# cmbant/getdist

Hardware: AMD Instinct MI355X
Metric: 2D KDE densities/sec (triangle, 50 params, 1e+07 samples) (higher is better)
Workload: dtype f64

## Files before the change

### getdist_amd/_lib.py

```python

import ctypes as C
import os
import subprocess

import numpy as np

_HERE = os.path.dirname(os.path.abspath(__file__))
LIB_PATH = os.path.join(_HERE, "csrc", "libgdhip.so")

GD_OK, GD_ERR_BADARG, GD_ERR_NOMEM, GD_ERR_HIP, GD_ERR_EMPTY, GD_ERR_SOLVER, GD_ERR_FFT, GD_ERR_NODEVICE, GD_ERR_TIMEOUT = \
    0, -1, -2, -3, -4, -5, -6, -7, -8


class GdhipError(RuntimeError):
    def __init__(self, code, msg):
        super().__init__("libgdhip error %d: %s" % (code, msg))
        self.code = code


class GdhipTimeout(GdhipError):
    """GD_ERR_TIMEOUT: a collective or the communicator set-up gave up waiting for a peer; the library has aborted and dropped
    the communicator, so the ranks renegotiate over the host application's own channel (parallel.init_library_comm)."""


def build_native(force=False):
    script = os.path.join(_HERE, "csrc", "build.sh")
    if force:
        for f in os.listdir(os.path.join(_HERE, "csrc")):
            if f.endswith(".o") or f.endswith(".so"):
                os.remove(os.path.join(_HERE, "csrc", f))
    subprocess.run(["bash", script], check=True)
    return LIB_PATH


_p = C.c_void_p
_i32, _i64, _f64 = C.c_int32, C.c_int64, C.c_double
_pd = C.POINTER(C.c_double)
_pi32 = C.POINTER(C.c_int32)
_pi64 = C.POINTER(C.c_int64)

SIGNATURES = {
    "gd_device_count": (C.c_int, []),
    "gd_create": (C.c_int, [C.c_int, C.POINTER(_p)]),
    "gd_destroy": (None, [_p]),
    "gd_last_error": (C.c_char_p, [_p]),
    "gd_version": (C.c_char_p, []),
    "gd_device_info": (C.c_int, [_p, _pi64]),
    "gd_sync": (C.c_int, [_p]),
    "gd_dev_alloc": (C.c_int, [_p, _i64, C.POINTER(_p)]),
    "gd_dev_free": (C.c_int, [_p, _p]),
    "gd_memcpy_h2d": (C.c_int, [_p, _p, _p, _i64]),
    "gd_memcpy_d2h": (C.c_int, [_p, _p, _p, _i64]),
    "gd_memcpy_d2h_async": (C.c_int, [_p, _p, _p, _i64]),
    "gd_copy_sync": (C.c_int, [_p]),
    "gd_memcpy_d2d": (C.c_int, [_p, _p, _p, _i64]),
    "gd_memset": (C.c_int, [_p, _p, C.c_int, _i64]),
    "gd_gather_items": (C.c_int, [_p, _p, _p, _pi32, _i32, _i64]),
    "gd_host_alloc": (C.c_int, [_p, _i64, C.POINTER(_p)]),
    "gd_host_free": (C.c_int, [_p, _p]),
    "gd_kde_lag_sums_2d": (C.c_int, [_p, _i32, _i32, _pd, _pi64, _i32, _pd]),
    "gd_autocov_lags_batch": (C.c_int, [_p, _pi32, _i32, _pd, _i64, _i32, _pd]),
    "gd_kde_lag_sums_batch": (C.c_int, [_p, _pi32, _i32, _pd, _pi64, _i32, _pd]),
    "gd_autocov_lags_range_batch": (C.c_int, [_p, _pi32, _i32, _pd, _i64, _i64, _i64, _i32, _pd]),
    "gd_timer_start": (C.c_int, [_p]),
    "gd_timer_stop_ms": (C.c_int, [_p, _pd]),
    "gd_upload": (C.c_int, [_p, _p, _i64, _i64, _i64, _i64, _p]),
    "gd_num_rows": (C.c_int, [_p, _pi64, _pi64]),
    "gd_column_ptr": (C.c_int, [_p, _i64, C.POINTER(_p)]),
    "gd_weight_stats": (C.c_int, [_p, _i64, _i64, _f64, _pd]),
    "gd_col_stats": (C.c_int, [_p, _i64, _i64, _pd]),
    "gd_cov": (C.c_int, [_p, _pi32, _i32, _i64, _i64, _pd, _pd, _pd, _pd]),
    "gd_quantiles": (C.c_int, [_p, _pi32, _i32, _i64, _i64, _pd, _i32, _pd]),
    "gd_quantiles_mm_probe": (C.c_int, [_p, _pi32, _i32, _i64, _i64, _pd, _i32, _pd, _pd, _pd, _pd, C.POINTER(C.c_int32)]),
    "gd_quantiles_mm": (C.c_int, [_p, _pi32, _i32, _i64, _i64, _pd, _i32, _pd, _pd]),
    "gd_autocov_lags": (C.c_int, [_p, _i32, _f64, _i64, _i32, _pd]),
    "gd_kde_lag_sums": (C.c_int, [_p, _i32, _f64, _pi64, _i32, _pd]),
    "gd_hist1d": (C.c_int, [_p, _pi32, _i32, _pd, _pd, _i32, _pd]),
    "gd_hist1d_dev": (C.c_int, [_p, _pi32, _i32, _pd, _pd, _i32, _p]),
    "gd_bin_indices": (C.c_int, [_p, _i32, _f64, _f64, _i32, _i32, _pi32, _pi64]),
    "gd_prebin": (C.c_int, [_p, _i32, _f64, _f64, _i32, _p]),
    "gd_prebin_batch": (C.c_int, [_p, _pi32, _i32, _pd, _pd, _i32, C.POINTER(_p)]),
    "gd_prebin8_batch": (C.c_int, [_p, _pi32, _i32, _pd, _pd, _i32, C.POINTER(_p), _pi64]),
    "gd_hist2d_prebinned8": (C.c_int, [_p, _i32, C.POINTER(_p), C.POINTER(_p), _p]),
    "gd_prebin8_hist2d": (C.c_int, [_p, _pi32, _i32, _pd, _pd, C.POINTER(_p), _pi64, _i32, C.POINTER(_p), C.POINTER(_p), _p]),
    "gd_hist2d": (C.c_int, [_p, _i32, _pi32, _pi32, _pd, _pd, _pd, _pd, _i32, _p]),
    "gd_hist2d_prebinned": (C.c_int, [_p, _i32, C.POINTER(_p), C.POINTER(_p), _i32, _p]),
    "gd_minmax_affine": (C.c_int, [_p, _i32, _pi32, _pi32, _pd, _pd, _pd]),
    "gd_hist2d_sheared": (C.c_int, [_p, _i32, _pi32, _pi32, _pd, _pd, _pd, _pd, _pd, _pd, _i32, _p]),
    "gd_dct1d": (C.c_int, [_p, _i32, _i32, _pd, _pd]),
    "gd_isj1d": (C.c_int, [_p, _i32, _i32, _pd, _pd, _pd, _pi32]),
    "gd_isj1d_dev": (C.c_int, [_p, _i32, _i32, _p, _pd, _pd, _pi32]),
    "gd_density1d": (C.c_int, [_p, _i32, _i32, _pd, _pd, _pi32, _pi32, _i32, _i32, _pd, _pi32]),
    "gd_density1d_dev": (C.c_int, [_p, _i32, _i32, _p, _pd, _pi32, _pi32, _i32, _i32, _pd, _pi32]),
    "gd_density1d_batch": (C.c_int, [_p, _p, _p, _i32, _pi32, _i32, _pd, _pd, _pd]),
    "gd_kopt2d": (C.c_int, [_p, _i32, _i32, _p, _pd, _pi32, _pd, _pd, _pd]),
    "gd_kopt2d_enqueue": (C.c_int, [_p, _i32, _i32, _p, _pd, _pi32, _pd, _pd, _p, _pi32]),
    "gd_kopt2d_finish": (C.c_int, [_p, _p, _i32, _i32, _p, _pd]),
    "gd_get_h": (C.c_int, [_p, _i32, _pd, _pd, _pd, _pi32, _pd]),
    "gd_density2d": (C.c_int, [_p, _i32, _i32, _p, _pd, _pd, _pd, _pi32, _pi32, _i32, _i32, _p, _pi32]),
    "gd_copy_mark": (C.c_int, [_p, _pi32]),
    "gd_copy_wait": (C.c_int, [_p, _i32]),
    "gd_density2d_enqueue": (C.c_int, [_p, _i32, _i32, _p, _pd, _pd, _pd, _pi32, _pi32, _i32, _i32, _p, _p]),
    "gd_density2d_enqueue_indexed": (C.c_int, [_p, _i32, _i32, _p, _pi32, _pd, _pd, _pd, _pi32, _pi32, _i32, _i32, _p, _p]),
    "gd_attach_samples": (C.c_int, [_p, _p]),
    "gd_bind_thread": (C.c_int, [_p]),
    "gd_contour_levels": (C.c_int, [_p, _i32, _i32, _p, _pd, _i32, _pd, _pi32]),
    "gd_limits1d": (C.c_int, [_p, _i32, _i32, _pd, _pd, _pd, _pd, _i32, _i32, _pd, _pi32]),
    "gd_set_extra_column": (C.c_int, [_p, _i32, _pd]),
    "gd_aux_weights": (C.c_int, [_p, _pd]),
    "gd_col_minmax": (C.c_int, [_p, _pi32, _i32, _i64, _i64, _i32, C.c_double, _pd]),
    "gd_weights_integral": (C.c_int, [_p, _pi32]),
    "gd_thin_rows": (C.c_int, [_p, _i64, _i64, _i64, _i32, _p, _i64, C.POINTER(C.c_int64)]),
    "gd_binary_transitions": (C.c_int, [_p, _pi32, _i32, _p, _i64, _pd, _i32, C.POINTER(C.c_int64)]),
    "gd_thinned_lag_sums": (C.c_int, [_p, _pi32, _i32, _pd, _p, _i64, _i32, _pd]),
    "gd_density2d_masked": (C.c_int, [_p, _i32, _p, C.c_double, C.c_double, C.c_double, _i32, _i32, _i32, _i32, _pd, _pd,
                                      C.POINTER(C.c_ubyte), _p, _pi32]),
    "gd_like_weights": (C.c_int, [_p, _pd, _i32, C.c_double, _pd]),
    "gd_select_weights": (C.c_int, [_p, _i32]),
    "gd_likes1d": (C.c_int, [_p, _i32, _i32, _pd, _pd, _pd, _pd, _pi32, _pi32, _i32, _pd, _pi32]),
    "gd_likes2d": (C.c_int, [_p, _i32, _i32, _p, _p, _pd, _pd, _pd, _pi32, _pi32, _i32, _p, _pi32]),
    "gd_circ_convolve": (C.c_int, [_p, _i32, _i32, _pd, _pd, _pd]),
    "gd_convolve1d_direct": (C.c_int, [_p, _pd, _i64, _pd, _i64, _pd]),
    "gd_autoconvolve": (C.c_int, [_p, _i32, _f64, _i32, _pd, _i64, _i64, _i64, _i32, _pd]),
    "gd_like_stats": (C.c_int, [_p, _i32, _pd]),
    "gd_batch2d_grid_sizes": (C.c_int, [_p, _i32, _pd, _pi32, _i32, _pi32]),
    "gd_density2d_batch": (C.c_int, [_p, _p, _p, _p, _i32, _pd, _pd, _pd, _pi32, _i32, _p, _p, _p, _i64, _pi32, _pd, _pd, _pi32,
                                     _pi32]),
    "gd_comm_unique_id": (C.c_int, [_p]),
    "gd_comm_init": (C.c_int, [_p, _i32, _i32, _p]),
    "gd_comm_info": (C.c_int, [_p, _pi32, _pi32]),
    "gd_comm_destroy": (C.c_int, [_p]),
    "gd_comm_abandon": (C.c_int, [_p]),
    "gd_comm_allgather": (C.c_int, [_p, _pd, _i64, _pd]),
    "gd_comm_allreduce_sum": (C.c_int, [_p, _pd, _i64]),
    "gd_comm_allgather_dev": (C.c_int, [_p, _p, _i64, _p]),
    "gd_comm_allreduce_sum_dev": (C.c_int, [_p, _p, _i64, _p]),
    "gd_batch2d_finish": (C.c_int, [_p]),
    "gd_batch2d_invalidate": (C.c_int, [_p]),
    "gd_batch2d_exchanges": (C.c_int, [_p, C.POINTER(C.c_int64)]),
    "gd_comm_rccl_path": (C.c_int, [C.c_char_p, C.c_int32, C.POINTER(C.c_int32)]),
    "gd_upload_shard": (C.c_int, [_p, _p, _i64, _i64, _i64, _i64, _i64, _p]),
    "gd_comm_share_columns": (C.c_int, [_p, C.POINTER(C.c_int64)]),
    "gd_histnd_batch": (C.c_int, [_p, _i32, _pi32, _pi32, _pd, _pd, _i32, _i32, _i32, _pd, _pd, _pd]),
    "gd_pca_corr": (C.c_int, [_p, _pi32, _i32, _pi32, _pd, _pd, _pd]),
    "gd_pca_project": (C.c_int, [_p, _pi32, _i32, _pi32, _pd, _pd, _pd, _i32, _i32, _pd, _pd, _pd, _pd, _pd, _pd]),
    "gd_mixture_nll": (C.c_int, [_p, _pi32, _i32, _i32, _pd, _pd, _pd, _i64, _i64, _pd]),
}

GD_HISTND_MAXD, GD_HISTND_MAX_BINS = 25, 1 << 25
GD_HISTND_H, GD_HISTND_LIKES, GD_HISTND_LMIN = 1, 2, 4
GD_PCA_MAX_PROJ = 448

_lib = None


def load_library():
    global _lib
    if _lib is None:
        if not os.path.exists(LIB_PATH):
            raise ImportError("libgdhip.so is not built: run `python -c 'import __graft_entry__ as g; g.build()'` "
                              "or getdist_amd/csrc/build.sh (there is no CPU fallback)")
        lib = C.CDLL(LIB_PATH)
        for name, (res, args) in SIGNATURES.items():
            fn = getattr(lib, name)
            fn.restype = res
            fn.argtypes = args
        _lib = lib
    return _lib


def _dp(a):
    return a.ctypes.data_as(_pd)


def _ip(a):
    return a.ctypes.data_as(_pi32)


def _f64arr(a):
    return np.ascontiguousarray(a, dtype=np.float64)


def _i32arr(a):
    return np.ascontiguousarray(a, dtype=np.int32)


class DevBuf:

    def __init__(self, ctx, nbytes):
        self.ctx = ctx
        self.nbytes = int(nbytes)
        self.ptr, self.capacity = ctx._take_block(self.nbytes)

    def free(self):
        if self.ptr and self.ctx.h:
            self.ctx._give_block(self.ptr, self.capacity)
        self.ptr = None

    def __del__(self):
        try:
            self.free()
        except Exception:
            pass

    def to_host(self, shape, dtype=np.float64, offset_bytes=0, pinned=False):
        out = self.ctx.pinned_array(shape, dtype) if pinned else np.empty(shape, dtype=dtype)
        self.ctx._check(self.ctx.lib.gd_memcpy_d2h(self.ctx.h, out.ctypes.data, self.ptr + offset_bytes, out.nbytes))
        return out

    def to_host_async(self, shape, dtype=np.float64):
        out = self.ctx.pinned_array(shape, dtype)
        self.ctx._check(self.ctx.lib.gd_memcpy_d2h_async(self.ctx.h, out.ctypes.data, self.ptr, out.nbytes))
        return out

    def from_host(self, arr, offset_bytes=0):
        arr = np.ascontiguousarray(arr)
        self.ctx._check(self.ctx.lib.gd_memcpy_h2d(self.ctx.h, self.ptr + offset_bytes, arr.ctypes.data, arr.nbytes))


class Context:

    def __init__(self, device=0):
        self.lib = load_library()
        self.h = None
        if self.lib.gd_device_count() <= 0:
            raise RuntimeError("getdist_amd needs a HIP device (no CPU fallback): none visible")
        h = _p()
        rc = self.lib.gd_create(int(device), C.byref(h))
        if rc != 0:
            raise GdhipError(rc, "gd_create(device=%d) failed" % device)
        self.h = h
        self.device = device
        self.N = self.n = 0
        self.weighted = False
        self._pinned = []
        self._free_blocks = []
        self._pinned_blocks = []
        self.comm_world = self.comm_rank = 0

    PINNED_POOL_LIMIT = 8 << 30

    def pinned_array(self, shape, dtype=np.float64):
        import sys

        nbytes = int(np.prod(shape)) * np.dtype(dtype).itemsize
        best = None
        for k, (ptr, nb, buf) in enumerate(self._pinned):
            if nb >= nbytes and sys.getrefcount(buf) <= 3 and (best is None or nb < self._pinned[best][1]):
                best = k
        if best is None:
# ... 475 lines not shown
        return buf, n.value

    def binary_transitions(self, cols, rows, K, thresholds):
        cols = _i32arr(cols)
        thresholds = _f64arr(thresholds).reshape(len(cols), -1)
        out = np.zeros((len(cols), thresholds.shape[1], 12), dtype=np.int64)
        self._check(self.lib.gd_binary_transitions(self.h, _ip(cols), len(cols), rows.ptr, int(K), _dp(thresholds),
                                                   thresholds.shape[1], out.ctypes.data_as(C.POINTER(C.c_int64))))
        return out

    def thinned_lag_sums(self, cols, means, rows, K, maxoff):
        cols, means = _i32arr(cols), _f64arr(means)
        out = np.zeros((len(cols), int(maxoff)))
        self._check(self.lib.gd_thinned_lag_sums(self.h, _ip(cols), len(cols), _dp(means), rows.ptr, int(K), int(maxoff),
                                                 _dp(out)))
        return out

    def like_weights(self, loglikes, mode, mean_loglike):
        if loglikes is None:
            self._check(self.lib.gd_like_weights(self.h, None, 0, 0.0, None))
            return None
        ll = _f64arr(loglikes)
        if ll.shape != (self.N,):
            raise ValueError("loglikes must have one entry per sample row")
        tot = C.c_double()
        self._check(self.lib.gd_like_weights(self.h, _dp(ll), int(mode), float(mean_loglike), C.byref(tot)))
        return tot.value

    def select_weights(self, which):
        self._check(self.lib.gd_select_weights(self.h, int(which)))

    def likes1d(self, hist, likehist, P, smooth, winw, flags, shade_mean_loglikes):
        hist, likehist, P = _f64arr(hist), _f64arr(likehist), _f64arr(P)
        B, F = hist.shape
        smooth, winw, flags = _f64arr(smooth), _i32arr(winw), _i32arr(flags)
        out = np.zeros_like(hist)
        status = np.zeros(B, dtype=np.int32)
        self._check(self.lib.gd_likes1d(self.h, B, F, _dp(hist), _dp(likehist), _dp(P), _dp(smooth), _ip(winw),
                                        _ip(flags), int(bool(shade_mean_loglikes)), _dp(out), _ip(status)))
        return out, status

    def likes2d(self, d_hist, d_likehist, B, F, rx, ry, corr, winw, flags, mbc):
        out = self.alloc(B * F * F * 8)
        rx, ry, corr, winw, flags = _f64arr(rx), _f64arr(ry), _f64arr(corr), _i32arr(winw), _i32arr(flags)
        status = np.zeros(B, dtype=np.int32)
        self._check(self.lib.gd_likes2d(self.h, B, F, d_hist.ptr, d_likehist.ptr, _dp(rx), _dp(ry), _dp(corr),
                                        _ip(winw), _ip(flags), int(mbc), out.ptr, _ip(status)))
        return out, status

    def circ_convolve(self, a, b):
        a, b = _f64arr(a), _f64arr(b)
        if a.shape != b.shape or a.ndim not in (1, 2):
            raise ValueError("circ_convolve needs two arrays of one shape, one- or two-dimensional")
        n0, n1 = (1, a.shape[0]) if a.ndim == 1 else a.shape
        out = np.empty_like(a)
        self._check(self.lib.gd_circ_convolve(self.h, int(n0), int(n1), _dp(a), _dp(b), _dp(out)))
        return out

    def convolve1d_direct(self, x, y):
        x, y = _f64arr(x), _f64arr(y)
        out = np.empty(x.size + y.size - 1)
        self._check(self.lib.gd_convolve1d_direct(self.h, _dp(x), x.size, _dp(y), y.size, _dp(out)))
        return out

    def autoconvolve(self, s, n, normalize=True, x=None, col=-1, mean=0.0, use_weights=False):
        out = np.empty(int(n))
        xx = None if x is None else _f64arr(x)
        self._check(self.lib.gd_autoconvolve(self.h, int(col), float(mean), int(bool(use_weights)),
                                             None if xx is None else _dp(xx), 0 if xx is None else xx.size, int(s), int(n),
                                             int(bool(normalize)), _dp(out)))
        return out

    def like_stats(self, col):
        out = np.zeros(8)
        self._check(self.lib.gd_like_stats(self.h, int(col), _dp(out)))
        return dict(min=out[0], max=out[1], norm=out[2], sum_wl=out[3], sum_wl2=out[4], sum_w_exp_plus=out[5],
                    sum_w_exp_minus=out[6], argmin=int(out[7]))

    def batch2d_grid_sizes(self, settings, n, corr, pairs32):
        F = np.zeros(len(pairs32), dtype=np.int32)
        rc = self.lib.gd_batch2d_grid_sizes(C.byref(settings), int(n), _dp(corr), _ip(pairs32), len(pairs32), _ip(F))
        if rc != 0:
            raise GdhipError(rc, "gd_batch2d_grid_sizes: bad argument")
        return F

    def density2d_batch(self, twin, settings, params, n, corr, cov, lag_probe, pairs32, exchange, grids, status, meta, levels,
                        level_status):
        tokens = np.full(2, -1, dtype=np.int32)
        self._check(self.lib.gd_density2d_batch(
            self.h, None if twin is None else twin.h, C.byref(settings), C.cast(params, _p), int(n), _dp(corr), _dp(cov),
            None if lag_probe is None else _dp(lag_probe), _ip(pairs32), len(pairs32),
            None if exchange is None else C.cast(exchange, _p), None, grids.ctypes.data, int(grids.size),
            status.ctypes.data_as(_pi32), _dp(meta), None if levels is None else _dp(levels),
            None if level_status is None else _ip(level_status), _ip(tokens)))
        return int(tokens[0]), int(tokens[1])

    @staticmethod
    def comm_unique_id():
        buf = C.create_string_buffer(128)
        rc = load_library().gd_comm_unique_id(buf)
        if rc != 0:
            raise GdhipError(rc, "gd_comm_unique_id failed (librccl.so missing?)")
        return buf.raw

    def comm_init(self, world, rank, id128):
        self._check(self.lib.gd_comm_init(self.h, int(world), int(rank), C.create_string_buffer(bytes(id128), 128)))
        self.comm_world, self.comm_rank = int(world), int(rank)

    def comm_allgather(self, vec):
        v = _f64arr(vec).ravel()
        out = np.empty((self.comm_world, v.size))
        self._check(self.lib.gd_comm_allgather(self.h, _dp(v), v.size, _dp(out)))
        return out

    def comm_allreduce_sum(self, vec):
        v = _f64arr(vec).ravel().copy()
        self._check(self.lib.gd_comm_allreduce_sum(self.h, _dp(v), v.size))
        return v

    def comm_destroy(self):
        self._check(self.lib.gd_comm_destroy(self.h))
        self.comm_world = 0

    def comm_info(self):
        wd, rk = C.c_int32(0), C.c_int32(0)
        self._check(self.lib.gd_comm_info(self.h, C.byref(wd), C.byref(rk)))
        return int(wd.value), int(rk.value)

    def comm_abandon(self):
        if self.h is not None:
            self.lib.gd_comm_abandon(self.h)

    def density1d_batch(self, settings, params, n, cols32, want_hist=False):
        cols32 = _i32arr(cols32)
        B, F = len(cols32), int(settings.fine_bins)
        P = np.zeros((B, F))
        hist = np.zeros((B, F)) if want_hist else None
        meta = np.zeros((B, 9))
        self._check(self.lib.gd_density1d_batch(self.h, C.byref(settings), C.cast(params, _p), int(n), _ip(cols32), B, _dp(P),
                                                None if hist is None else _dp(hist), _dp(meta)))
        return P, hist, meta

    def batch2d_finish(self):
        self._check(self.lib.gd_batch2d_finish(self.h))

    def batch2d_invalidate(self):
        self._check(self.lib.gd_batch2d_invalidate(self.h))

    def batch2d_exchanges(self):
        c = C.c_int64(0)
        self._check(self.lib.gd_batch2d_exchanges(self.h, C.byref(c)))
        return int(c.value)

    def kopt2d(self, d_hist, B, F, neff, do_corr, fallback_t, corr):
        neff, do_corr, fallback_t, corr = _f64arr(neff), _i32arr(do_corr), _f64arr(fallback_t), _f64arr(corr)
        out = np.zeros((B, 12))
        self._check(self.lib.gd_kopt2d(self.h, B, F, d_hist.ptr if isinstance(d_hist, DevBuf) else d_hist, _dp(neff),
                                       _ip(do_corr), _dp(fallback_t), _dp(corr), _dp(out)))
        return out

    def get_h(self, psi, neff, corr, do_corr):
        psi, neff, corr, do_corr = _f64arr(psi).reshape(-1, 6), _f64arr(neff), _f64arr(corr), _i32arr(do_corr)
        out = np.zeros((len(psi), 4))
        self._check(self.lib.gd_get_h(self.h, len(psi), _dp(psi), _dp(neff), _dp(corr), _ip(do_corr), _dp(out)))
        return out

    def density2d(self, d_hist, B, F, rx, ry, corr, winw, flags, bco, mbc, out=None):
        out = out or self.alloc(B * F * F * 8)
        rx, ry, corr, winw, flags = _f64arr(rx), _f64arr(ry), _f64arr(corr), _i32arr(winw), _i32arr(flags)
        status = np.zeros(B, dtype=np.int32)
        self._check(self.lib.gd_density2d(self.h, B, F, d_hist.ptr if isinstance(d_hist, DevBuf) else d_hist, _dp(rx),
                                          _dp(ry), _dp(corr), _ip(winw), _ip(flags), int(bco), int(mbc), out.ptr,
                                          _ip(status)))
        return out, status
```

### getdist_amd/csrc/batch2d.hip

```cpp
#include "batch1d.hpp"
#include "batch2d.hpp"
#include "ctx.hpp"

namespace {

gd_ctx* C(void* h) { return (gd_ctx*)h; }

const gdb::Ops kOps = {
     [](void* h) { return gd_bind_thread(C(h)); },
     [](void* h, int64_t* N, int64_t* n) { return gd_num_rows(C(h), N, n); },
    [](void* h, int32_t* hw) {
        gd_ctx* c = C(h);
        *hw = c->w == nullptr ? 0 : ((!c->w8 && !c->w_integral && c->w_sum > 1e-200 && c->w_sum < 1e200) ? 2 : 1);
        return 0;
    },
     [](void* h, int64_t bytes, void** out) { return gd_dev_alloc(C(h), bytes, out); },
     [](void* h, void* p) { return gd_dev_free(C(h), p); },
    [](void* h, const int32_t* cols, int32_t ncols, const double* binmin, const double* width, int32_t F, void* const* d_idx,
       int64_t* bad) { return gd_prebin8_batch(C(h), cols, ncols, binmin, width, F, d_idx, bad); },
    [](void* h, int32_t B, const void* const* ix, const void* const* iy, void* d_hist) {
        return gd_hist2d_prebinned8(C(h), B, ix, iy, d_hist);
    },
    [](void* h, const int32_t* cols, int32_t ncols, const double* binmin, const double* width, void* const* d_idx, int64_t* bad,
       int32_t B, const void* const* ix, const void* const* iy, void* d_hist) {
        return gd_prebin8_hist2d(C(h), cols, ncols, binmin, width, d_idx, bad, B, ix, iy, d_hist);
    },
    [](void* h, int32_t col, double binmin, double width, int32_t F, void* d_idx) {
        return gd_prebin(C(h), col, binmin, width, F, d_idx);
    },
    [](void* h, int32_t B, const void* const* ix, const void* const* iy, int32_t F, void* d_hist) {
        return gd_hist2d_prebinned(C(h), B, ix, iy, F, d_hist);
    },
    [](void* h, int32_t B, const int32_t* ci, const int32_t* cj, const double* a, const double* b, double* out) {
        return gd_minmax_affine(C(h), B, ci, cj, a, b, out);
    },
    [](void* h, int32_t B, const int32_t* ci, const int32_t* cj, const double* r0, const double* r1, const double* xmin,
       const double* dx, const double* ymin, const double* dy, int32_t F, void* d_hist) {
        return gd_hist2d_sheared(C(h), B, ci, cj, r0, r1, xmin, dx, ymin, dy, F, d_hist);
    },
    [](void* h, int32_t B, int32_t F, const void* d_hist, const double* neff, const int32_t* do_corr, const double* fallback_t,
       const double* corr, double* out) { return gd_kopt2d(C(h), B, F, d_hist, neff, do_corr, fallback_t, corr, out); },
    [](void* h, void* d_dst, int64_t dst_first, const void* d_src, const int32_t* index, int32_t count, int64_t item_bytes) {
        return gd_gather_items(C(h), (char*)d_dst + dst_first * item_bytes, d_src, index, count, item_bytes);
    },
    [](void* h, int32_t B, int32_t F, const void* d_hist, const int32_t* hist_index, const double* rx, const double* ry,
       const double* corr, const int32_t* winw, const int32_t* flags, int32_t bco, int32_t mbc, void* d_P, int32_t* status_pinned) {
        return gd_density2d_enqueue_indexed(C(h), B, F, d_hist, hist_index, rx, ry, corr, winw, flags, bco, mbc, d_P, status_pinned);
    },
     [](void* h, void* dst, const void* d_src, int64_t bytes) { return gd_memcpy_d2h_async(C(h), dst, d_src, bytes); },
     [](void* h, int32_t* token) { return gd_copy_mark(C(h), token); },
    [](void* h, int32_t token) {
        if (!gd_ctx_alive(C(h))) return 0;
        const int rc = gd_copy_wait(C(h), token);
        return rc == GD_ERR_BADARG ? 0 : rc;
    },
     [](void* h) { return gd_ctx_alive(C(h)) ? gd_copy_sync(C(h)) : 0; },
    [](void* h, int32_t B, int32_t F, const void* d_P, const double* contours, int32_t nc, double* out, int32_t* status) {
        return gd_contour_levels(C(h), B, F, d_P, contours, nc, out, status);
    },
    [](void* h, const int32_t* cols, int32_t ncols, const double* means, int64_t k0, int32_t nlags, double* out) {
        return gd_autocov_lags_batch(C(h), cols, ncols, means, k0, nlags, out);
    },
    [](void* h, const int32_t* cols, int32_t ncols, const double* inv4s2, const int64_t* lags, int32_t nlags, double* out) {
        return gd_kde_lag_sums_batch(C(h), cols, ncols, inv4s2, lags, nlags, out);
    },
    [](void* h, int32_t col, double inv4s2, const int64_t* lags, int32_t nlags, double* out) {
        return gd_kde_lag_sums(C(h), col, inv4s2, lags, nlags, out);
    },
     [](void* h) { return gd_last_error(C(h)); },
    [](void* h, void** aux) {
        gd_ctx* a = nullptr;
        int rc = gd_create(C(h)->device, &a);
        if (rc == 0) rc = gd_attach_samples(a, C(h));
        if (rc == 0) rc = gd_stream_priority(a, 1);
        if (rc) {
            if (a) gd_destroy(a);
            return gd_fail(C(h), rc, "could not create the third context of a batched call");
        }
        *aux = a;
        return 0;
    },
    [](void* aux) {
        gd_destroy(C(aux));
        return 0;
    },
    [](void* h, int32_t B, int32_t F, const void* d_hist, const double* neff, const int32_t* do_corr, const double* fallback_t,
       const double* corr, void* d_rows, int32_t* ticket) {
        return gd_kopt2d_enqueue(C(h), B, F, d_hist, neff, do_corr, fallback_t, corr, d_rows, ticket);
    },
    [](void* h, void* stage_a_h, int32_t ticket, int32_t B, void* d_rows, double* out) {
        return gd_kopt2d_finish(C(h), C(stage_a_h), ticket, B, d_rows, out);
    },
     [](void* h) { return C(h)->comm ? C(h)->comm_world : 0; },
     [](void* h, double* inout, int64_t count) { return gd_comm_allreduce_sum(C(h), inout, count); },
     [](void* ctx, int level) { return gd_stream_priority(C(ctx), level); },
    [](void* h, const int32_t* cols, int32_t ncols, const double* binmin, const double* width, int32_t F, void* const* d_idx) {
        return gd_prebin_batch(C(h), cols, ncols, binmin, width, F, d_idx);
    },
};

const gdb::Ops1D kOps1D = {
    [](void* h, const int32_t* cols, int32_t ncols, const double* binmin, const double* width, int32_t F, void* d_hist) {
        return gd_hist1d_dev(C(h), cols, ncols, binmin, width, F, d_hist);
    },
    [](void* h, int32_t B, int32_t F, const void* d_hist, const double* neff, double* hfrac, int32_t* status) {
        return gd_isj1d_dev(C(h), B, F, d_hist, neff, hfrac, status);
    },
    [](void* h, int32_t B, int32_t F, const void* d_hist, const double* smooth, const int32_t* winw, const int32_t* flags,
       int32_t bco, int32_t mbc, double* P_out, int32_t* status) {
        return gd_density1d_dev(C(h), B, F, d_hist, smooth, winw, flags, bco, mbc, P_out, status);
    },
    [](void* h, void* dst, const void* d_src, int64_t bytes) {
        const int rc = gd_fetch(C(h), dst, d_src, (size_t)bytes);
        return rc ? rc : gd_stream_sync(C(h));
    },
};

void release_state(gd_ctx* ctx, bool destroy) {
    gdb::State* st = (gdb::State*)ctx->batch_state;
    if (!st) return;
    gdb::release_all(*st, kOps, ctx);
    if (destroy) {
        delete st;
        ctx->batch_state = nullptr;
    }
}

gdb::State& state_of(gd_ctx* ctx) {
    if (!ctx->batch_state) {
        ctx->batch_state = new gdb::State();
        ctx->batch_state_release = release_state;
    }
    return *(gdb::State*)ctx->batch_state;
}

}

extern "C" {

int gd_batch2d_grid_sizes(const gd_batch2d_settings* settings, int32_t n, const double* corr, const int32_t* pairs, int32_t P,
                          int32_t* F_out) {
    if (!settings || !corr || (!pairs && P > 0) || (!F_out && P > 0) || n <= 0 || P < 0) return GD_ERR_BADARG;
    for (int k = 0; k < 2 * P; ++k)
        if (pairs[k] < 0 || pairs[k] >= n) return GD_ERR_BADARG;
    gdb::PairScalars ps;
    gdb::pair_scalars(*settings, n, corr, pairs, P, ps);
    for (int k = 0; k < P; ++k) F_out[k] = ps.F[k];
    return GD_OK;
}

int gd_density2d_batch(gd_ctx* ctx, gd_ctx* twin, const gd_batch2d_settings* settings, gd_param2d* params, int32_t n,
                       const double* corr, const double* cov, const double* lag_probe, const int32_t* pairs, int32_t P,
                       gd_neff_exchange_fn exchange, void* exchange_user, void* grids_pinned, int64_t grids_doubles,
                       int32_t* status_pinned, double* meta, double* levels, int32_t* level_status, int32_t* tokens_out2) {
    GD_REQUIRE(ctx && settings && params && corr && cov && tokens_out2 && n > 0 && P >= 0, "bad argument");
    GD_REQUIRE(P == 0 || (pairs && grids_pinned && status_pinned && meta), "bad argument");
    GD_REQUIRE(ctx->cols, "no samples uploaded");
    GD_REQUIRE(!twin || (twin != ctx && twin->cols == ctx->cols), "the second context must be attached to the first (gd_attach_samples)");
    GD_REQUIRE(ctx->w_sel == 0, "auxiliary weights are selected");
    GD_REQUIRE(!settings->want_levels || (settings->contours && settings->ncontours > 0 && levels && level_status), "contour levels requested without room for them");
    GD_HIP(hipSetDevice(ctx->device));
    int rc;
    try {
        gdb::Call call(state_of(ctx), kOps, ctx, twin, *settings, params, n, corr, cov, lag_probe, pairs, P, exchange, exchange_user,
                       (double*)grids_pinned, grids_doubles, status_pinned, meta, levels, level_status);
        rc = call.run(tokens_out2);
        if (rc) ctx->err = call.err;
    } catch (const std::exception& e) {
        rc = gd_fail(ctx, GD_ERR_NOMEM, "gd_density2d_batch: %s", e.what());
    }
    return rc;
}

int gd_density1d_batch(gd_ctx* ctx, const gd_density1d_settings* settings, gd_param2d* params, int32_t n, const int32_t* cols,
                       int32_t B, double* P_out, double* hist_out, double* meta) {
    GD_REQUIRE(ctx && settings && params && cols && P_out && meta && n > 0 && B > 0, "bad argument");
    GD_REQUIRE(ctx->cols, "no samples uploaded");
    GD_REQUIRE(ctx->w_sel == 0, "auxiliary weights are selected");
    GD_HIP(hipSetDevice(ctx->device));
    int rc;
    try {
        std::string err;
        rc = gdb::density1d_batch(state_of(ctx), kOps, kOps1D, ctx, *settings, params, n, cols, B, P_out, hist_out, meta, &err);
        if (rc) ctx->err = err;
    } catch (const std::exception& e) {
        rc = gd_fail(ctx, GD_ERR_NOMEM, "gd_density1d_batch: %s", e.what());
    }
    return rc;
}

int gd_batch2d_finish(gd_ctx* ctx) {
    GD_REQUIRE(ctx, "null context");
    if (!ctx->batch_state) return GD_OK;
    GD_HIP(hipSetDevice(ctx->device));
    return gdb::finish_all(*(gdb::State*)ctx->batch_state, kOps, ctx);
}

int gd_batch2d_exchanges(gd_ctx* ctx, int64_t* count_out) {
    GD_REQUIRE(ctx && count_out, "null argument");
    *count_out = 0;
    if (ctx->batch_state) {
        gdb::State& st = *(gdb::State*)ctx->batch_state;
        std::lock_guard<std::mutex> g(st.mu);
        *count_out = st.exchanges_entered;
    }
    return GD_OK;
}

int gd_batch2d_invalidate(gd_ctx* ctx) {
    GD_REQUIRE(ctx, "null context");
    if (!ctx->batch_state) return GD_OK;
    gdb::invalidate_index_columns(*(gdb::State*)ctx->batch_state);
    return GD_OK;
}

}
```

### getdist_amd/csrc/batch2d.hpp

```cpp
#pragma once
#include <math.h>
#include <stdint.h>
#include <stdio.h>
#include <stdlib.h>
#include <string.h>
#include <time.h>

#include <algorithm>
#include <atomic>
#include <chrono>
#include <condition_variable>
#include <deque>
#include <functional>
#include <future>
#include <map>
#include <mutex>
#include <string>
#include <thread>
#include <vector>

#include "../../include/gdhip.h"

namespace gdb {

struct Ops {
    int (*bind_thread)(void* h);
    int (*num_rows)(void* h, int64_t* N, int64_t* n);
    int (*weights_kind)(void* h, int32_t* has_weights);
    int (*dev_alloc)(void* h, int64_t bytes, void** out);
    int (*dev_free)(void* h, void* p);
    int (*prebin8_batch)(void* h, const int32_t* cols, int32_t ncols, const double* binmin, const double* width, int32_t F,
                         void* const* d_idx, int64_t* bad);
    int (*hist2d_prebinned8)(void* h, int32_t B, const void* const* ix, const void* const* iy, void* d_hist);
    int (*prebin8_hist2d)(void* h, const int32_t* cols, int32_t ncols, const double* binmin, const double* width,
                          void* const* d_idx, int64_t* bad, int32_t B, const void* const* ix, const void* const* iy, void* d_hist);
    int (*prebin)(void* h, int32_t col, double binmin, double width, int32_t F, void* d_idx);
    int (*hist2d_prebinned)(void* h, int32_t B, const void* const* ix, const void* const* iy, int32_t F, void* d_hist);
    int (*minmax_affine)(void* h, int32_t B, const int32_t* ci, const int32_t* cj, const double* a, const double* b, double* out);
    int (*hist2d_sheared)(void* h, int32_t B, const int32_t* ci, const int32_t* cj, const double* r0, const double* r1,
                          const double* xmin, const double* dx, const double* ymin, const double* dy, int32_t F, void* d_hist);
    int (*kopt2d)(void* h, int32_t B, int32_t F, const void* d_hist, const double* neff, const int32_t* do_corr,
                  const double* fallback_t, const double* corr, double* out);
    int (*gather_items)(void* h, void* d_dst, int64_t dst_first, const void* d_src, const int32_t* index, int32_t count,
                        int64_t item_bytes);
    int (*density2d_enqueue)(void* h, int32_t B, int32_t F, const void* d_hist, const int32_t* hist_index, const double* rx,
                             const double* ry, const double* corr, const int32_t* winw, const int32_t* flags, int32_t bco,
                             int32_t mbc, void* d_P, int32_t* status_pinned);
    int (*d2h_async)(void* h, void* dst, const void* d_src, int64_t bytes);
    int (*copy_mark)(void* h, int32_t* token);
    int (*copy_wait)(void* h, int32_t token);
    int (*copy_sync)(void* h);
    int (*contour_levels)(void* h, int32_t B, int32_t F, const void* d_P, const double* contours, int32_t nc, double* out,
                          int32_t* status);
    int (*autocov_lags_batch)(void* h, const int32_t* cols, int32_t ncols, const double* means, int64_t k0, int32_t nlags,
                              double* out);
    int (*kde_lag_sums_batch)(void* h, const int32_t* cols, int32_t ncols, const double* inv4s2, const int64_t* lags,
                              int32_t nlags, double* out);
    int (*kde_lag_sums)(void* h, int32_t col, double inv4s2, const int64_t* lags, int32_t nlags, double* out);
    const char* (*last_error)(void* h);
    int (*create_aux)(void* h, void** aux);
    int (*destroy_aux)(void* aux);
    int (*kopt2d_enqueue)(void* h, int32_t B, int32_t F, const void* d_hist, const double* neff, const int32_t* do_corr,
                          const double* fallback_t, const double* corr, void* d_rows, int32_t* ticket);
    int (*kopt2d_finish)(void* h, void* stage_a_h, int32_t ticket, int32_t B, void* d_rows, double* out);
    int (*comm_world)(void* h);
    int (*comm_allreduce_sum)(void* h, double* inout, int64_t count);
    int (*stream_priority)(void* ctx, int level);
    int (*prebin_batch)(void* h, const int32_t* cols, int32_t ncols, const double* binmin, const double* width, int32_t F,
                        void* const* d_idx);
};

static inline double py_pow(double x, double y) {
    volatile double e = y;
    return pow(x, e);
}
static inline double np_minimum(double a, double b) { return (a < b || isnan(a)) ? a : b; }
static inline double np_maximum(double a, double b) { return (a > b || isnan(a)) ? a : b; }
static inline double np_sign(double x) { return isnan(x) ? x : (x > 0 ? 1.0 : (x < 0 ? -1.0 : 0.0)); }

static inline int frame_size(int n) {
    long long best = 1LL << 40;
    const int odd[5] = {1, 3, 5, 9, 15};
    for (int a = 4; a < 28; ++a)
        for (int q = 0; q < 5; ++q) {
            const long long v = (1LL << a) * odd[q];
            if (v >= n && v < best) best = v;
        }
    return (int)best;
}

static inline bool chol_shear(double c00, double c10, double c11, double S[4], double r[2]) {
    if (!(c00 > 0)) return false;
    const double l00 = sqrt(c00);
    const double l10 = c10 * (1.0 / l00);
    const double d = c11 - l10 * l10;
    if (!(d > 0)) return false;
    const double l11 = sqrt(d);
    double i00, i10, i11;
    if (fabs(l10) > fabs(l00)) {
        const double l = l00 * (1.0 / l10);
        const double u11 = 0.0 - l * l11;
        i10 = 1.0 * (1.0 / u11);
        i00 = (0.0 - l11 * i10) * (1.0 / l10);
        i11 = (0.0 - l * 1.0) * (1.0 / u11);
    } else {
        const double l = l10 * (1.0 / l00);
        i00 = 1.0 * (1.0 / l00);
        i10 = (0.0 - l * 1.0) * (1.0 / l11);
        i11 = 1.0 * (1.0 / l11);
    }
    S[0] = l00 * i00, S[1] = 0.0 * i00, S[2] = l10 * i00, S[3] = l11 * i00;
    r[0] = i10 / i00, r[1] = i11 / i00;
    return true;
}

struct PairScalars {
    std::vector<int32_t> jx, jy, F, warn;
    std::vector<int64_t> nbin2D;
    std::vector<double> actual, corr;
};

static inline void pair_scalars(const gd_batch2d_settings& s, int n, const double* corrmat, const int32_t* pairs, int P,
                                PairScalars& ps) {
    ps.jx.resize(P), ps.jy.resize(P), ps.F.resize(P), ps.warn.assign(P, 0), ps.nbin2D.resize(P), ps.actual.resize(P),
        ps.corr.resize(P);
    const int base_F = s.fine_bins_2D;
    for (int k = 0; k < P; ++k) {
        const int a = pairs[2 * k], b = pairs[2 * k + 1];
        ps.jx[k] = a, ps.jy[k] = b;
        const double actual = corrmat[(size_t)b * n + a];
        double c = actual;
        if (fabs(fabs(c) - 1.0) <= 1e-8) {
            ps.warn[k] |= 1;
            c = np_sign(c) * s.max_corr_2D;
        }
        if (fabs(c) < 0.1) c = 0.0;
        const double m = np_minimum(s.max_corr_2D, fabs(c));
        const double angle_scale = np_maximum(0.2, sqrt(1 - m * m));
        ps.nbin2D[k] = (int64_t)nearbyint((double)s.num_bins_2D / angle_scale);
        const int64_t scaled = 192 * (int64_t)(3 / angle_scale) / 3;
        ps.F[k] = (c != 0 && base_F < scaled && (int64_t)(1 / angle_scale) > 1) ? (int32_t)scaled : base_F;
        ps.actual[k] = actual, ps.corr[k] = c;
    }
}

static inline void bin_edges(const gd_param2d& p, double* binmin, double* binmax) {
    const double border = (p.range_max - p.range_min) * 0.1;
    double lo = np_minimum(p.param_min, p.range_min);
    if (!p.has_limits_bot) lo = lo - border;
    double hi = np_maximum(p.param_max, p.range_max);
    if (!p.has_limits_top) hi = hi + border;
    *binmin = lo, *binmax = hi;
}

struct NeffInput {
    int64_t N;
    double norm, sum_w2;
};

static inline int neff_from_lags(const NeffInput& in, int64_t maxoff, double min_corr, const double* sums, int nseed_tail,
                                 const std::function<int(int64_t, double*)>& lag_sum, double* neff_out) {
    const int64_t N = in.N;
    if (maxoff > N / 10) maxoff = N / 10;
    const int64_t uncorr_len = N / 2;
    int64_t nav = 0;
    for (int64_t k = uncorr_len; k < uncorr_len + 5; ++k) nav += N - k;
    double s5 = 0.0;
    for (int q = 0; q < 5; ++q) s5 += sums[q];
    const double uncorr_term = s5 / (double)nav;
    const double n = (double)N;
    std::map<int64_t, double> cache;
    for (int q = 0; q < nseed_tail; ++q) cache[q + 1] = sums[5 + q];
    int rc = 0;
    auto corr_k = [&](int64_t k) -> double {
        auto it = cache.find(k);
        double v;
        if (it == cache.end()) {
            v = NAN;
            const int e = lag_sum(k, &v);
            if (e) rc = e;
            cache[k] = v;
        } else {
            v = it->second;
        }
        return v - (n - (double)k) * uncorr_term;
    };
    const double corr0 = in.sum_w2;
    const double threshold = min_corr * corr0;
    const double c1 = corr_k(1);
    double Nn;
    if (c1 < threshold) {
        Nn = corr0;
    } else {
        const double c2 = corr_k(2);
        if (c2 > threshold) {
            int64_t max_k = maxoff;
            while (max_k > 10) {
                if (corr_k(max_k / 3) >= threshold) break;
                max_k /= 3;
            }
            const int64_t step_size = max_k < 20 ? 1 : max_k / 10;
            double cum_sum = c1 + c2;
            for (int64_t k = 3; k < maxoff + 1; k += step_size) {
                const double test_val = corr_k(k);
                if (test_val < threshold) break;
                cum_sum += k > 3 ? test_val * (double)step_size : (test_val * (double)step_size) / 2;
            }
            Nn = corr0 + 2 * cum_sum;
        } else {
            Nn = corr0 + 2 * c1;
        }
    }
    if (rc) return rc;
    *neff_out = py_pow(in.norm, 2.0) / Nn;
    return 0;
}

struct Plan {
    std::vector<int8_t> branch;
    std::vector<uint8_t> has_limits;
    std::vector<double> rangex, rangey, ratio, neff, fallback_t;
    std::vector<int32_t> si, sj;
    std::vector<uint8_t> swap, has_imin, has_imax;
    std::vector<double> imin, imax, S, r;
// ... 51 lines not shown
    void* ptr = nullptr;
    double binmin = NAN, width = NAN;
    bool valid = false;
};

struct Pending {
    std::vector<void*> blocks;
    int32_t tok_main = -1, tok_twin = -1;
    void* twin = nullptr;
    bool live = false;
};

struct State {
    std::mutex mu;
    std::vector<std::pair<void*, int64_t>> free_blocks;
    std::map<void*, int64_t> capacity;
    int64_t cached_bytes = 0;
    std::map<std::tuple<int, int, int>, IdxCol> idx;
    Pending prev;
    void* aux = nullptr;
    void* aux2 = nullptr;
    int64_t exchanges_entered = 0;
    static constexpr int64_t kCacheLimit = 16LL << 30;
};

struct Pool {
    State& st;
    const Ops& ops;
    void* h;
    void* take(int64_t bytes, int* rc) {
        {
            std::lock_guard<std::mutex> g(st.mu);
            int best = -1;
            for (size_t k = 0; k < st.free_blocks.size(); ++k) {
                const int64_t cap = st.free_blocks[k].second;
                if (cap >= bytes && cap <= 2 * bytes + (1 << 20) && (best < 0 || cap < st.free_blocks[best].second)) best = (int)k;
            }
            if (best >= 0) {
                void* p = st.free_blocks[best].first;
                st.cached_bytes -= st.free_blocks[best].second;
                st.free_blocks.erase(st.free_blocks.begin() + best);
                return p;
            }
        }
        void* p = nullptr;
        int e = ops.dev_alloc(h, bytes, &p);
        if (e == GD_ERR_NOMEM) {
            drop_cached();
            e = ops.dev_alloc(h, bytes, &p);
        }
        if (e) {
            *rc = e;
            return nullptr;
        }
        std::lock_guard<std::mutex> g(st.mu);
        st.capacity[p] = bytes;
        return p;
    }
    void give(void* p) {
        if (!p) return;
        std::unique_lock<std::mutex> g(st.mu);
        const int64_t cap = st.capacity[p];
        if (st.cached_bytes + cap > State::kCacheLimit) {
            st.capacity.erase(p);
            g.unlock();
            ops.dev_free(h, p);
            return;
        }
        st.free_blocks.emplace_back(p, cap);
        st.cached_bytes += cap;
    }
    void drop_cached() {
        std::vector<std::pair<void*, int64_t>> blocks;
        {
            std::lock_guard<std::mutex> g(st.mu);
            blocks.swap(st.free_blocks);
            st.cached_bytes = 0;
            for (auto& b : blocks) st.capacity.erase(b.first);
        }
        for (auto& b : blocks) ops.dev_free(h, b.first);
    }
};

static inline int complete_pending(State& st, const Ops& ops, void* h, Pending& pd) {
    if (!pd.live) return 0;
    int rc = 0;
    if (pd.tok_main >= 0) rc = ops.copy_wait(h, pd.tok_main);
    if (!rc && pd.twin && pd.tok_twin >= 0) rc = ops.copy_wait(pd.twin, pd.tok_twin);
    Pool pool{st, ops, h};
    for (void* p : pd.blocks) pool.give(p);
    pd.blocks.clear();
    pd.live = false;
    return rc;
}

static inline int finish_all(State& st, const Ops& ops, void* h) { return complete_pending(st, ops, h, st.prev); }

static inline void invalidate_index_columns(State& st) {
    std::lock_guard<std::mutex> g(st.mu);
    for (auto& kv : st.idx) kv.second.valid = false;
}

static inline void release_all(State& st, const Ops& ops, void* h) {
    finish_all(st, ops, h);
    Pool pool{st, ops, h};
    {
        std::lock_guard<std::mutex> g(st.mu);
        for (auto& kv : st.idx)
            if (kv.second.ptr) st.free_blocks.emplace_back(kv.second.ptr, st.capacity[kv.second.ptr]);
        st.idx.clear();
    }
    pool.drop_cached();
    if (st.aux) {
        ops.destroy_aux(st.aux);
        st.aux = nullptr;
    }
    if (st.aux2) {
        ops.destroy_aux(st.aux2);
        st.aux2 = nullptr;
    }
}

struct Call {
    State& st;
    const Ops& ops;
    void* h;
    void* twin;
    const gd_batch2d_settings& s;
    gd_param2d* par;
    int n;
    const double* corrmat;
    const double* cov;
    const double* lag_probe;
    const int32_t* pairs;
    int P;
    gd_neff_exchange_fn exchange;
    void* exchange_user;
    double* grids;
    int64_t grids_doubles;
    int32_t* status_pinned;
    double* meta;
    double* levels;
    int32_t* level_status;
    std::string err;

    Call(State& st_, const Ops& ops_, void* h_, void* twin_, const gd_batch2d_settings& s_, gd_param2d* par_, int n_,
         const double* corr_, const double* cov_, const double* lag_probe_, const int32_t* pairs_, int P_,
         gd_neff_exchange_fn ex_, void* ex_user_, double* grids_, int64_t grids_doubles_, int32_t* status_, double* meta_,
         double* levels_, int32_t* level_status_)
        : st(st_), ops(ops_), h(h_), twin(twin_), s(s_), par(par_), n(n_), corrmat(corr_), cov(cov_), lag_probe(lag_probe_),
          pairs(pairs_), P(P_), exchange(ex_), exchange_user(ex_user_), grids(grids_), grids_doubles(grids_doubles_),
          status_pinned(status_), meta(meta_), levels(levels_), level_status(level_status_), pool{st_, ops_, h_} {}

    int64_t N = 0;
    bool unit_weights = true;
    Pool pool;
    PairScalars ps;
    std::vector<int> used;
    std::vector<double> bmin, bmax;
    std::vector<double> fwx, fwy;
    std::vector<int> F_list;
    std::map<int, std::vector<int>> classes;
    std::map<int, void*> hists;
    Plan plan;
    struct Shear {
        void* d_rot = nullptr;
        std::vector<int> A;
        std::vector<double> r1s, r2s;
    } shear;
    bool have_shear = false;
    bool byte_index_weights = false;
    std::vector<double> rx, ry, cc, smooth, W;
    std::vector<int64_t> winw;
    std::vector<int32_t> flags, group;
    std::vector<void*> call_blocks;
    std::vector<void*> bin_stale;
    std::mutex enq_mu;
    std::atomic<int> bin_launching{0};
    bool hold_neff_for_binning = false;
    std::atomic<int> bin_done{0};
    bool shear_after_binning = false;
    std::future<int> shear_future;
    bool shear_deferred = false;
    std::atomic<bool> shear_joined{true};
    std::mutex shear_mu;
    std::atomic<int> shear_hist_state{1};
    int shear_hist_rc = 0;
    std::atomic<int> first_part_done{0};
    static constexpr int32_t kStatusPending = 0x7fffffff;
    std::atomic<const volatile int32_t*> first_part_flag{nullptr};
    int reports_enqueued = 0;
    std::shared_future<int> bin_future;
    std::mutex bin_mu;
    std::atomic<int> bins_first_done{0};
    int bins_first_rows = 0;
    int bin_rc = 0;
    bool bin_joined = true;
    int join_binning() {
        std::lock_guard<std::mutex> g(bin_mu);
        if (!bin_joined) {
            bin_joined = true;
            bin_rc = bin_future.valid() ? bin_future.get() : 0;
            mark("binning: joined");
        }
        return bin_rc;
    }
    size_t base_part_size(size_t total, int F) const {
        size_t want = 2;
        if (const char* e = getenv("GDHIP_KOPT_PARTS")) want = (size_t)std::max(1, atoi(e));
        size_t part = std::max<size_t>((size_t)s_kopt_split_min(), (total + want - 1) / want);
        size_t align = 256;
        if (const char* e = getenv("GDHIP_KOPT_PART_ALIGN")) align = (size_t)std::max(0, atoi(e));
        if (align > 1 && F == 256 && part > align) part = std::max<size_t>(align, (part + align / 2 - 1) / align * align);
        return part;
    }
    static size_t first_part_size(size_t part) {
        if (const char* e = getenv("GDHIP_KOPT_FIRST_PART")) {
            const size_t f = (size_t)std::max(0, atoi(e));
            if (f > 0 && f < part) return f;
        }
        return part;
    }
    static int shear_hold_us() {
        const char* e = getenv("GDHIP_BATCH_SHEAR_HOLD_US");
        return e ? atoi(e) : 0;
    }
    int join_shear(bool release = false) {
        if (release) first_part_done.store(1);
        std::lock_guard<std::mutex> g(shear_mu);
        if (shear_joined.load()) return 0;
        const int e = shear_future.valid() ? shear_future.get() : 0;
        shear_joined.store(true);
        mark("shear: joined");
        return e;
    }
    int64_t grid_off = 0;
    int status_at = 0;
    int batch_no = 0;
    std::vector<void*> conv_ctxs;
    std::vector<int> side_classes;
    std::vector<int> order;

    std::mutex tl_mu;
    std::vector<std::pair<double, std::string>> tl;
    bool tl_on = getenv("GDHIP_BATCH_LOG") != nullptr;
    static double now_ms() {
        timespec ts;
        clock_gettime(CLOCK_MONOTONIC, &ts);
        return ts.tv_sec * 1e3 + ts.tv_nsec * 1e-6;
    }
    void mark(const char* what, int a = -1, int b = -1) {
        if (!tl_on) return;
        char buf[160];
        if (a >= 0 && b >= 0)
            snprintf(buf, sizeof buf, "%s (%d, %d)", what, a, b);
        else if (a >= 0)
            snprintf(buf, sizeof buf, "%s (%d)", what, a);
        else
            snprintf(buf, sizeof buf, "%s", what);
        std::lock_guard<std::mutex> g(tl_mu);
        tl.emplace_back(now_ms(), buf);
    }
    void dump_timeline() {
        if (!tl_on || tl.empty()) return;
        std::sort(tl.begin(), tl.end());
        fprintf(stderr, "---- gd_density2d_batch host timeline (ms)\n");
        for (auto& e : tl) fprintf(stderr, "%9.3f  %s\n", e.first - tl[0].first, e.second.c_str());
    }

    std::mutex err_mu;
    int fail(int code, const std::string& msg) {
        std::lock_guard<std::mutex> g(err_mu);
        if (err.empty()) err = msg;
        return code;
    }
    int dev_fail(int code, void* ctx) {
        const char* m = ops.last_error(ctx);
        return fail(code, m && *m ? m : "device call failed");
    }
#define GDB_DEV(ctx_, call_)                       \
    do {                                           \
        const int rc__ = (call_);                  \
        if (rc__) return dev_fail(rc__, (ctx_));   \
    } while (0)
#define GDB_TRY(call_)            \
    do {                          \
        const int rc__ = (call_); \
        if (rc__) return rc__;    \
    } while (0)

    double* M(int k) { return meta + (size_t)k * GD_BATCH2D_META; }

    int neff_batch(const std::vector<int>& js, bool owned_only, double min_corr = 0.05) {
        std::vector<int32_t> todo;
        for (int j : js)
            if (isnan(par[j].neff) && (!owned_only || (par[j].owned & 1))) todo.push_back(j);
        if (todo.empty()) return 0;
        mark("neff: start", (int)todo.size());
        if (s.uncorrelated_sampler) {
            for (int j : todo) par[j].neff = py_pow(s.norm, 2.0) / s.sum_w2;
            return 0;
        }
        const int m = (int)todo.size();
        const int64_t max_off = N / 10;
        const int nl = (int)std::min<int64_t>(8, max_off + 1);
        std::vector<double> lag0((size_t)m * nl);
// ... 354 lines not shown
        int64_t mb = (int64_t)(s_max_batch_bytes() / ((double)F * F * 8 * 30));
        int max_batch = (int)std::max<int64_t>(1, std::min<int64_t>(mb, s_max_batch()));
        const int first_batch = s_first_batch();
        std::vector<int> gorder;
        for (int q : pos_all) {
            const int g = group[members[q]];
            if (std::find(gorder.begin(), gorder.end(), g) == gorder.end()) gorder.push_back(g);
        }
        for (int g : gorder) {
            std::map<int, std::vector<int>> byS;
            for (int q : pos_all) {
                const int k = members[q];
                if (group[k] != g) continue;
                const int64_t w = winw[k];
                if (w < 1 || w > 2 * (int64_t)F) return fail(GD_ERR_BADARG, "bad window half-width");
                byS[frame_size(F + 2 * (int)w)].push_back(q);
            }
            for (auto& kv : byS) {
                const std::vector<int>& cur = kv.second;
                size_t s0 = 0;
                if (batches.empty() && (int)cur.size() > first_batch) {
                    Batch b;
                    b.pos.assign(cur.begin(), cur.begin() + first_batch);
                    batches.push_back(b);
                    s0 = first_batch;
                }
                for (size_t s1 = s0; s1 < cur.size(); s1 += max_batch) {
                    Batch b;
                    b.pos.assign(cur.begin() + s1, cur.begin() + std::min(cur.size(), s1 + (size_t)max_batch));
                    batches.push_back(b);
                }
            }
        }
        for (auto& b : batches)
            for (int q : b.pos) b.ks.push_back(members[q]);
        return 0;
    }
    int s_first_batch() const {
        if (s.first_batch > 0) return s.first_batch;
        const char* e = getenv("GDHIP_BATCH_FIRST_BATCH");
        return e && atoi(e) > 0 ? atoi(e) : 128;
    }
    int s_max_batch() const {
        if (s.max_batch > 0) return s.max_batch;
        const char* e = getenv("GDHIP_BATCH_MAX_BATCH");
        return e && atoi(e) > 0 ? atoi(e) : 320;
    }
    double s_max_batch_bytes() const { return s.max_batch_bytes > 0 ? s.max_batch_bytes : 24e9; }
    int s_two_min() const { return s.two_streams_min > 0 ? s.two_streams_min : 64; }
    int s_two_split() const { return s.two_streams_split > 0 ? s.two_streams_split : 400; }
    int s_kopt_split_min() const { return s.kopt_split_min > 0 ? s.kopt_split_min : 256; }

    bool is_side(int F) const { return std::find(side_classes.begin(), side_classes.end(), F) != side_classes.end(); }

    int enqueue_batch(int F, const Batch& b, void* force_ctx) {
        const std::vector<int>& members = classes.at(F);
        void* bctx;
        if (force_ctx)
            bctx = force_ctx;
        else if (!side_classes.empty() || P > s_two_split())
            bctx = conv_ctxs[is_side(F) && conv_ctxs.size() > 1 ? 1 : 0];
        else
            bctx = conv_ctxs[batch_no % conv_ctxs.size()];
        ++batch_no;
        const int B = (int)b.pos.size();
        const int64_t item = (int64_t)F * F * 8;
        void* d_hist;
        {
            std::lock_guard<std::mutex> g(enq_mu);
            d_hist = hists.at(F);
        }
        int rc = 0;
        bool whole = B == (int)members.size();
        for (int q = 0; q < B && whole; ++q) whole = b.pos[q] == q;
        std::vector<int32_t> hidx(b.pos.begin(), b.pos.end());
        std::vector<double> rxb(B), ryb(B), ccb(B);
        std::vector<int32_t> wb(B), fb(B);
        for (int q = 0; q < B; ++q) {
            const int k = b.ks[q];
            rxb[q] = rx[k], ryb[q] = ry[k], ccb[q] = cc[k], wb[q] = (int32_t)winw[k], fb[q] = flags[k];
        }
        void* d_P = pool.take((int64_t)B * item, &rc);
        if (!d_P) return dev_fail(rc, h);
        call_blocks.push_back(d_P);
        int32_t* status = status_pinned + status_at;
        for (int q = 0; q < B; ++q) status[q] = kStatusPending;
        if (grid_off + (int64_t)B * F * F > grids_doubles) return fail(GD_ERR_BADARG, "grids_pinned is too small");
        mark(bctx == h ? "conv: enqueue on main" : "conv: enqueue on twin", B, F);
        GDB_DEV(bctx, ops.density2d_enqueue(bctx, B, F, d_hist, whole ? nullptr : hidx.data(), rxb.data(), ryb.data(), ccb.data(),
                                            wb.data(), fb.data(), s.boundary_correction_order, s.mult_bias_correction_order, d_P,
                                            status));
        mark("conv: enqueued");
        if (s.want_levels && levels) {
            std::vector<double> lv((size_t)B * s.ncontours);
            std::vector<int32_t> ls(B);
            GDB_DEV(bctx, ops.contour_levels(bctx, B, F, d_P, s.contours, s.ncontours, lv.data(), ls.data()));
            for (int q = 0; q < B; ++q) {
                memcpy(levels + (size_t)b.ks[q] * s.ncontours, &lv[(size_t)q * s.ncontours], sizeof(double) * s.ncontours);
                level_status[b.ks[q]] = ls[q];
            }
        }
        GDB_DEV(bctx, ops.d2h_async(bctx, grids + grid_off, d_P, (int64_t)B * item));
        for (int q = 0; q < B; ++q) {
            double* m = M(b.ks[q]);
            m[1] = (double)(grid_off + (int64_t)q * F * F);
            m[29] = bctx == twin ? 1.0 : 0.0;
            m[30] = (double)(status_at + q);
        }
        grid_off += (int64_t)B * F * F;
        status_at += B;
        return 0;
    }

    int run_class(int F, const std::vector<char>& only, void* force_ctx) {
        std::vector<Batch> batches;
        GDB_TRY(class_batches(F, only, batches));
        for (const Batch& b : batches) GDB_TRY(enqueue_batch(F, b, force_ctx));
        return 0;
    }

    int enqueue_all() {
        std::vector<int> main_, side;
        for (int F : order) (is_side(F) ? side : main_).push_back(F);
        const std::vector<char> all;
        std::vector<Batch> first;
        size_t first_done = 0;
        if (!side.empty() && !main_.empty()) {
            GDB_TRY(class_batches(main_[0], all, first));
            if (!first.empty()) {
                GDB_TRY(enqueue_batch(main_[0], first[0], nullptr));
                first_done = 1;
            }
        }
        for (int F : side) GDB_TRY(run_class(F, all, nullptr));
        for (size_t q = 0; q < main_.size(); ++q) {
            if (q == 0 && !side.empty()) {
                for (size_t b = first_done; b < first.size(); ++b) GDB_TRY(enqueue_batch(main_[0], first[b], nullptr));
                continue;
            }
            GDB_TRY(run_class(main_[q], all, nullptr));
        }
        return 0;
    }

    struct Launch {
        int F = 0;
        std::vector<int> ks;
        int na = 0;
        void* d_hist = nullptr;
        std::vector<int> pos;
        bool whole = false;
        void* d_batch = nullptr;
        bool own = false;
        void* d_rows = nullptr;
        int32_t ticket = -1;
        std::vector<double> ne, fb, ci;
        std::vector<int32_t> dc;
    };
    typedef std::function<int(const std::vector<int>&, int, int)> ChunkFn;

    template <class BufFn>
    int ready_for(Launch& L, const BufFn& class_buffer) {
        if (L.na > 0 && L.d_hist && !shear_joined.load() && !getenv("GDHIP_BATCH_SHEAR_JOIN_WHOLE")) {
            while (shear_hist_state.load(std::memory_order_acquire) == 0) std::this_thread::sleep_for(std::chrono::microseconds(20));
            mark("shear: histograms awaited");
            if (shear_hist_state.load(std::memory_order_acquire) == 2) {
                (void)join_shear();
                return shear_hist_rc ? shear_hist_rc : GD_ERR_HIP;
            }
        } else if (L.na > 0 || !L.d_hist) {
            const int e = join_shear();
            if (e) return e;
            if (!L.d_hist) L.d_hist = class_buffer(L.F);
            if (!L.d_hist) return fail(GD_ERR_BADARG, "a grid-size class has no histograms");
        }
        return 0;
    }

    int build_batch(Launch& L) {
        const int B = (int)L.ks.size(), F = L.F;
        const int64_t item = (int64_t)F * F * 8;
        L.d_batch = L.d_hist, L.own = false;
        if (!L.whole) {
            int rc = 0;
            L.d_batch = pool.take((int64_t)B * item, &rc);
            if (!L.d_batch) return dev_fail(rc, h);
            L.own = true;
            if (L.na) {
                std::vector<int32_t> idx(L.na);
                for (int a = 0; a < L.na; ++a) idx[a] = a;
                GDB_DEV(h, ops.gather_items(h, L.d_batch, 0, shear.d_rot, idx.data(), L.na, item));
            }
            if (!L.pos.empty()) {
                std::vector<int32_t> idx(L.pos.begin(), L.pos.end());
                GDB_DEV(h, ops.gather_items(h, L.d_batch, L.na, L.d_hist, idx.data(), (int)idx.size(), item));
            }
        }
        L.ne.resize(B), L.fb.resize(B), L.ci.resize(B), L.dc.resize(B);
        for (int row = 0; row < B; ++row) {
            const int k = L.ks[row];
            const bool rowA = row < L.na;
            L.ne[row] = plan.neff[k], L.dc[row] = plan.has_limits[k] ? 0 : 1;
            L.fb[row] = rowA ? -1.0 : plan.fallback_t[k];
            L.ci[row] = rowA ? 0.0 : ps.actual[k];
        }
        return 0;
    }

    int absorb_rows(const Launch& L, const std::vector<double>& out) {
        const int B = (int)L.ks.size();
        for (int row = 0; row < B; ++row) {
            const double* o = &out[(size_t)row * 12];
            if (o[7] == 0 && o[11] != 0) return fail(GD_ERR_BADARG, "bias not positive definite");
        }
        for (int row = 0; row < B; ++row) {
            const int k = L.ks[row];
            const double* o = &out[(size_t)row * 12];
            memcpy(M(k) + 6, o, 12 * sizeof(double));
            double hx, hy, c;
            if (row < L.na) {
                const double hxa = o[8] * shear.r1s[row], hya = o[9] * shear.r2s[row], ca = o[10];
                const double* S = &plan.S[(size_t)4 * k];
                const double k00 = hxa * hxa, k01 = hxa * hya * ca, k11 = hya * hya;
                const double t00 = S[0] * k00 + S[1] * k01, t01 = S[0] * k01 + S[1] * k11;
                const double t10 = S[2] * k00 + S[3] * k01, t11 = S[2] * k01 + S[3] * k11;
                const double c00 = t00 * S[0] + t01 * S[1], c01 = t00 * S[2] + t01 * S[3], c11 = t10 * S[2] + t11 * S[3];
                const double sx = sqrt(c00), sy = sqrt(c11);
                hx = plan.swap[k] ? sy : sx, hy = plan.swap[k] ? sx : sy, c = c01 / sqrt(c00 * c11);
            } else {
                hx = o[8] * plan.rangex[k], hy = o[9] * plan.rangey[k], c = o[10];
            }
            if (o[7] != 0) {
                if (s.raise_on_bandwidth_errors) {
                    char buf[200];
                    snprintf(buf, sizeof buf, "2D kernel density bandwidth optimizer failed for pair %d (columns %d, %d). "
                             "Using fallback width: 2D fixed point: no root in [0, 0.1]", k, (int)ps.jx[k], (int)ps.jy[k]);
                    return fail(GD_ERR_SOLVER, buf);
                }
                ps.warn[k] |= 4;
                const double d = py_pow(plan.neff[k], 1.0 / 6);
                hx = par[ps.jx[k]].sigma_range / d, hy = par[ps.jy[k]].sigma_range / d;
                c = std::max(std::min(ps.actual[k], s.max_corr_2D), -s.max_corr_2D);
            }
            W[(size_t)3 * k] = hx, W[(size_t)3 * k + 1] = hy, W[(size_t)3 * k + 2] = c;
        }
        return 0;
    }

    static bool part_on_main(int index, int nparts) { return nparts > 1 && index >= nparts - std::max(1, 2 * nparts / 5); }

    int bandwidth_2d(bool staged, void* aux, const ChunkFn& on_chunk) {
        const int base_F = s.fine_bins_2D;
        const int m = s.mult_bias_correction_order;
        std::vector<double> widen;
        if (m) {
            widen.resize(P);
            const double e = 1.0 / 6 - 1.0 / (2 + 4 * (1 + m));
            for (int k = 0; k < P; ++k) widen[k] = 1.1 * py_pow(plan.neff[k], e);
        }
        if (!have_shear && !shear_deferred) GDB_TRY(shear_histograms(h));
        std::vector<int> A;
        for (int k = 0; k < P; ++k)
            if (plan.branch[k] == 0) A.push_back(k);
        const int nA = (int)A.size();
        auto class_buffer = [&](int F) -> void* {
            std::lock_guard<std::mutex> g(enq_mu);
            auto it = hists.find(F);
            return it == hists.end() ? nullptr : it->second;
        };
        std::vector<int> waiting;
        for (int k = 0; k < P; ++k)
            if (plan.branch[k] == 1) {
                const double c = std::max(std::min(ps.actual[k], s.max_corr_2D), -s.max_corr_2D);
                const double d = py_pow(plan.neff[k], 1.0 / 6);
                W[(size_t)3 * k] = par[ps.jx[k]].sigma_range / d, W[(size_t)3 * k + 1] = par[ps.jy[k]].sigma_range / d, W[(size_t)3 * k + 2] = c;
                waiting.push_back(k);
            }
        std::vector<Launch> launches;
        bool merged = false;
        for (int F : F_list) {
            const std::vector<int>& mem = classes.at(F);
            std::vector<int> pos_C;
            for (int q = 0; q < (int)mem.size(); ++q)
                if (plan.branch[mem[q]] == 2) pos_C.push_back(q);
            if (F == base_F && !pos_C.empty()) {
                const size_t total = pos_C.size() + (size_t)nA;
                size_t part = total;
                if (staged && (int)pos_C.size() >= s_kopt_split_min()) part = base_part_size(total, F);
                const size_t nparts = shear_deferred ? std::max<size_t>(1, (total + part - 1) / part) : 0;
                for (size_t c0 = 0, first = 1, ip = 0; c0 < pos_C.size(); first = 0, ++ip) {
                    Launch L;
                    const bool carries = shear_deferred ? (ip + 1 == nparts || pos_C.size() - c0 <= part) : first != 0;
                    L.F = F, L.na = carries ? nA : 0, L.d_hist = class_buffer(F);
                    const size_t part_q = (ip == 0 && nparts > 1) ? first_part_size(part) : part;
                    size_t take_ = std::min(pos_C.size() - c0, part_q > (size_t)L.na ? part_q - (size_t)L.na : (size_t)1);
                    if (shear_deferred && carries) take_ = pos_C.size() - c0;
                    L.pos.assign(pos_C.begin() + c0, pos_C.begin() + c0 + take_);
                    c0 += take_;
                    L.whole = L.na == 0 && L.pos.size() == mem.size();
                    for (int q = 0; q < L.na; ++q) L.ks.push_back(A[q]);
                    for (int q : L.pos) L.ks.push_back(mem[q]);
                    launches.push_back(std::move(L));
                }
                merged = true;
                continue;
            }
            if (pos_C.empty()) continue;
            Launch L;
            L.F = F, L.na = 0, L.d_hist = class_buffer(F), L.pos = pos_C, L.whole = pos_C.size() == mem.size();
            for (int q : pos_C) L.ks.push_back(mem[q]);
            launches.push_back(std::move(L));
        }
        if (nA && !merged) {
            GDB_TRY(join_shear(true));
            Launch L;
            L.F = base_F, L.na = nA, L.d_hist = shear.d_rot, L.whole = true;
            L.ks = A;
            launches.push_back(std::move(L));
        }
        const int nl = (int)launches.size();
        if (!staged || nl == 0 || launches[0].na > 0 || !launches[0].d_hist) first_part_done.store(1);
        auto report = [&](std::vector<int> ks, int index) -> int {
            if (!waiting.empty()) {
                std::vector<int> all, later;
                for (int k : waiting) ((shear_deferred && ps.F[k] != base_F && index + 1 < nl) ? later : all).push_back(k);
                all.insert(all.end(), ks.begin(), ks.end());
                ks.swap(all);
                waiting.swap(later);
            }
            if (m)
                for (int k : ks) W[(size_t)3 * k] *= widen[k], W[(size_t)3 * k + 1] *= widen[k];
            if (shear_deferred && index + 1 >= nl) {
                const int e = join_shear();
                if (e) return e;
            }
            if (!ks.empty() || index + 1 >= nl) return on_chunk(ks, index, nl);
            return 0;
        };
        int rc = 0;
        auto rows_binned_first = [&](const Launch& L) {
            if (bins_first_rows <= 0 || L.F != base_F || L.na > 0 || !L.d_hist) return false;
            for (int q : L.pos)
                if (q >= bins_first_rows) return false;
            return true;
        };
        auto whole_binning_for = [&](Launch& L) -> int {
            const int e = join_binning();
            if (e) return e;
            if (L.F == base_F && !L.pos.empty())
                if (void* p = class_buffer(L.F)) L.d_hist = p;
            return 0;
        };
        if (!staged || nl == 0) {
            rc = join_binning();
            for (int q = 0; q < nl && !rc; ++q) {
                Launch& L = launches[q];
                const int B = (int)L.ks.size();
                rc = whole_binning_for(L);
                if (!rc) rc = ready_for(L, class_buffer);
                if (!rc) rc = build_batch(L);
                std::vector<double> out((size_t)B * 12);
                if (!rc) {
                    mark("kopt: launch", B, L.F);
                    rc = ops.kopt2d(h, B, L.F, L.d_batch, L.ne.data(), L.dc.data(), L.fb.data(), L.ci.data(), out.data());
                    mark("kopt: done");
                    if (rc) dev_fail(rc, h);
                }
                if (L.own) pool.give(L.d_batch);
                if (!rc) rc = absorb_rows(L, out);
                if (!rc) rc = report(L.ks, q);
            }
            if (!rc && nl == 0) rc = report({}, 0);
        } else {
            std::mutex mu;
            std::condition_variable cv;
            int n_staged = 0;
            bool abort_ = false;
            std::deque<int> handed;
            std::future<int> enqueuer = std::async(std::launch::async, [&]() -> int {
                ops.bind_thread(h);
                int e = 0;
                for (;;) {
                    int q;
                    {
                        std::unique_lock<std::mutex> g(mu);
                        cv.wait(g, [&] { return !handed.empty(); });
                        q = handed.front();
                        handed.pop_front();
                    }
                    if (q < 0) return e;
                    if (e) continue;
                    if (part_on_main(q, nl) || !shear_deferred) {
                        std::unique_lock<std::mutex> g(mu);
                        cv.wait(g, [&] { return n_staged >= nl || abort_; });
                        if (n_staged < nl) {
                            e = GD_ERR_HIP;
                            continue;
                        }
                    }
                    e = join_binning();
                    if (!e) e = report(launches[q].ks, q);
                    if (reports_enqueued++ == 0 && status_at > 0 && !s.results_in_flight && !getenv("GDHIP_BATCH_SHEAR_ON_ENQUEUE"))
                        first_part_flag.store(status_pinned + status_at - 1);
                    first_part_done.store(1);
                }
            });
            std::future<int> finisher = std::async(std::launch::async, [&]() -> int {
                ops.bind_thread(aux);
                int e = 0;
                auto hand = [&](int q) {
                    std::lock_guard<std::mutex> g(mu);
                    handed.push_back(q);
                    cv.notify_all();
                };
                for (int q = 0; q < nl; ++q) {
                    {
                        std::unique_lock<std::mutex> g(mu);
                        cv.wait(g, [&] { return n_staged > q || abort_; });
                        if (n_staged <= q) break;
                    }
                    Launch& L = launches[q];
                    const int B = (int)L.ks.size();
                    std::vector<double> out((size_t)B * 12);
                    if (!e) {
                        e = ops.kopt2d_finish(aux, h, L.ticket, B, L.d_rows, out.data());
                        mark("kopt: part finished", q, B);
                        if (e) dev_fail(e, aux);
                    } else {
                        ops.copy_sync(h);
                    }
                    if (L.own) pool.give(L.d_batch);
                    pool.give(L.d_rows);
                    if (!e) e = absorb_rows(L, out);
                    if (e || getenv("GDHIP_BATCH_SHEAR_AFTER_GET_H")) first_part_done.store(1);
                    if (!e) hand(q);
                }
                first_part_done.store(1);
                hand(-1);
                return e;
            });
            for (int q = 0; q < nl && !rc; ++q) {
                Launch& L = launches[q];
                const int B = (int)L.ks.size();
                if (!(q == 0 && rows_binned_first(L))) rc = whole_binning_for(L);
                if (!rc) rc = ready_for(L, class_buffer);
                if (!rc) rc = build_batch(L);
                if (!rc) {
                    L.d_rows = pool.take((int64_t)B * GD_KOPT_BLOCK_DOUBLES * 8, &rc);
                    if (!L.d_rows) dev_fail(rc, h);
                }
                if (!rc) {
                    mark("kopt: stage A enqueue", q, B);
                    rc = ops.kopt2d_enqueue(h, B, L.F, L.d_batch, L.ne.data(), L.dc.data(), L.fb.data(), L.ci.data(), L.d_rows, &L.ticket);
                    if (rc) dev_fail(rc, h);
                }
                std::lock_guard<std::mutex> g(mu);
                if (rc) {
                    abort_ = true;
                    if (L.own && L.d_batch) ops.copy_sync(h), pool.give(L.d_batch);
                    if (L.d_rows) pool.give(L.d_rows);
                } else {
                    ++n_staged;
                }
                cv.notify_all();
            }
            {
                std::lock_guard<std::mutex> g(mu);
                if (n_staged < nl) abort_ = true;
                cv.notify_all();
            }
            mark("kopt: every stage A enqueued");
            const int e = finisher.get();
            const int e2 = enqueuer.get();
            if (!rc) rc = e;
            if (!rc) rc = e2;
        }
        {
            const int e0 = join_binning();
            const int e = join_shear(true);
            if (!rc) rc = e0;
            if (!rc) rc = e;
        }
        if (shear.d_rot) pool.give(shear.d_rot), shear.d_rot = nullptr;
        return rc;
    }

    int run(int32_t* tokens_out2) {
        tokens_out2[0] = tokens_out2[1] = -1;
        const int base_F = s.fine_bins_2D, bco = s.boundary_correction_order;
        const double ss = s.smooth_scale_2D;
        if (fabs(s.max_corr_2D) > 1) return fail(GD_ERR_BADARG, "max_corr_2D cannot be >=1");
        if (bco > 1) return fail(GD_ERR_BADARG, "unknown boundary_correction_order (expected 0 or 1)");
        if (base_F < 8 || base_F > 4096) return fail(GD_ERR_BADARG, "fine_bins_2D out of range");
        bool exchanged = false;
        if (P == 0) {
            GDB_TRY(neff_exchange(&exchanged));
            return 0;
        }
        mark("call: start", P);
        int64_t ncols = 0;
        GDB_DEV(h, ops.num_rows(h, &N, &ncols));
        if (ncols < n) return fail(GD_ERR_BADARG, "more parameters than resident columns");
        int32_t hw = 0;
        GDB_DEV(h, ops.weights_kind(h, &hw));
        unit_weights = hw == 0;
        byte_index_weights = hw == 2 && !getenv("GDHIP_NO_WSORT");
        for (int k = 0; k < P; ++k)
            if (pairs[2 * k] < 0 || pairs[2 * k] >= n || pairs[2 * k + 1] < 0 || pairs[2 * k + 1] >= n)
                return fail(GD_ERR_BADARG, "pair index out of range");
        {
            std::vector<char> seen(n, 0);
            for (int k = 0; k < 2 * P; ++k)
                if (!seen[pairs[k]]) seen[pairs[k]] = 1, used.push_back(pairs[k]);
        }
        const bool injected = ss < 0 && s.bandwidths != nullptr;
        const bool auto_bw = ss < 0 && !injected;
        bool need_neff = false;
        if (auto_bw && !s.pair_neff)
            for (int j : used) need_neff = need_neff || isnan(par[j].neff);
        void* aux = nullptr;
        const bool overlap = auto_bw && P >= 64 && twin != nullptr;
        if (overlap) {
            if (!st.aux) GDB_DEV(h, ops.create_aux(h, &st.aux));
            aux = st.aux;
        }
        std::future<int> neff_f, shear_f;
        bin_launching.store(0);
        hold_neff_for_binning = overlap && need_neff && unit_weights && !getenv("GDHIP_BATCH_NO_NEFF_HOLD");
        if (overlap && need_neff)
            neff_f = std::async(std::launch::async, [this] {
                ops.bind_thread(h);
                return neff_batch(used, true);
            });
        bmin.assign(n, NAN), bmax.assign(n, NAN);
        for (int j : used) bin_edges(par[j], &bmin[j], &bmax[j]);
        pair_scalars(s, n, corrmat, pairs, P, ps);
        fwx.resize(P), fwy.resize(P);
        for (int k = 0; k < P; ++k) {
            const int F = ps.F[k];
            if (!classes.count(F)) F_list.push_back(F);
            classes[F].push_back(k);
            fwx[k] = (bmax[ps.jx[k]] - bmin[ps.jx[k]]) / (F - 1);
            fwy[k] = (bmax[ps.jy[k]] - bmin[ps.jy[k]]) / (F - 1);
            double* m = M(k);
            for (int q = 0; q < GD_BATCH2D_META; ++q) m[q] = NAN;
            m[0] = F, m[5] = -1, m[23] = bmin[ps.jx[k]], m[24] = bmax[ps.jx[k]], m[25] = bmin[ps.jy[k]], m[26] = bmax[ps.jy[k]];
            m[27] = ps.corr[k], m[28] = (double)ps.nbin2D[k];
        }
        int64_t need = 0;
        for (int k = 0; k < P; ++k) need += (int64_t)ps.F[k] * ps.F[k];
        if (need > grids_doubles && !s.bandwidths_only) {
            if (neff_f.valid()) neff_f.get();
            return fail(GD_ERR_BADARG, "grids_pinned is too small");
        }
        std::vector<double> rngx(P), rngy(P);
        for (int k = 0; k < P; ++k) rngx[k] = bmax[ps.jx[k]] - bmin[ps.jx[k]], rngy[k] = bmax[ps.jy[k]] - bmin[ps.jy[k]];
        int rc = 0;
        if (auto_bw) {
            if (overlap) {
                const bool split_classes = F_list.size() > 1;
                bin_done.store(0);
                first_part_done.store(0);
                first_part_flag.store(nullptr), reports_enqueued = 0;
                {
                    const char* e = getenv("GDHIP_BATCH_SHEAR_DEFERRED");
                    const char* emin = getenv("GDHIP_BATCH_SHEAR_DEFERRED_MIN");
                    shear_deferred = (e ? atoi(e) != 0 : true) && unit_weights && P >= (emin ? atoi(emin) : 256);
                    if (shear_deferred && !st.aux2) {
                        int rc2 = ops.create_aux(h, &st.aux2);
                        if (!rc2 && ops.stream_priority && getenv("GDHIP_BATCH_SHEAR_LOW_PRIORITY")) rc2 = ops.stream_priority(st.aux2, -1);
                        if (rc2) {
                            if (st.aux2) ops.destroy_aux(st.aux2), st.aux2 = nullptr;
                            shear_deferred = false, (void)ops.last_error(h);
                        }
                    }
                    shear_after_binning = shear_deferred;
                }
                rc = make_plan(s, par, n, cov, ps, rngx, rngy, 0.2, plan, err);
                bins_first_rows = 0;
                bins_first_done.store(0);
                const bool will_stage = aux != nullptr && !s.want_levels && P >= s_two_min() && P > s_two_split() && !s.bandwidths_only;
                if (!rc && shear_deferred && will_stage && base_F == 256 && main_class() == 256 && !getenv("GDHIP_BATCH_ONE_BINNING")) {
                    std::vector<int>& mem = classes[256];
                    std::stable_partition(mem.begin(), mem.end(), [&](int k) { return plan.branch[k] == 2; });
                    size_t nC = 0, nA = 0;
                    for (int k : mem) nC += plan.branch[k] == 2;
                    for (int k = 0; k < P; ++k) nA += plan.branch[k] == 0;
                    if ((int)nC >= s_kopt_split_min()) {
                        const size_t part = base_part_size(nC + nA, 256), first = std::min(nC, first_part_size(part));
                        if (nC + nA > part && first < mem.size()) bins_first_rows = (int)first;
                    }
                }
                bin_joined = false, bin_rc = 0;
                bin_future = std::async(std::launch::async, [this, split_classes] {
                                 ops.bind_thread(twin);
                                 const int e = binning(twin, split_classes ? 1 : 0);
                                 bins_first_done.store(1);
                                 bin_done.store(1);
                                 return e;
                             }).share();
                if (!rc) shear_hist_state.store(0);
                if (!rc)
                    shear_f = std::async(std::launch::async, [this, aux, split_classes] {
                        void* sctx = shear_deferred ? st.aux2 : aux;
                        ops.bind_thread(sctx);
                        if (shear_after_binning) {
// ... 183 lines not shown
```

### getdist_amd/csrc/ctx.hpp

```cpp
#pragma once
#include <hip/hip_runtime.h>
#include <stdint.h>
#include <stdio.h>
#include <string.h>

#include <map>
#include <memory>
#include <mutex>
#include <set>
#include <string>
#include <atomic>
#include <vector>

#include "../../include/gdhip.h"

struct FftPlanCache;

struct BucketCols {
    std::mutex mu;
    unsigned short* buf = nullptr;
    int64_t n = 0, ld = 0;
    bool tried = false;
    std::vector<double> mn, scale;
    std::vector<int> nb;
    ~BucketCols() {
        if (buf) (void)hipFree(buf);
    }
};

#define GD_EXTRA_COLS 4

struct gd_ctx {
    int device = 0;
    hipStream_t stream = nullptr;
    hipStream_t copy_stream = nullptr;
    hipEvent_t copy_ev = nullptr;
    bool main_high = false;
    hipEvent_t ev0 = nullptr, ev1 = nullptr;
    int cu_count = 256;
    std::string err;
    double* cols = nullptr;
    double* w = nullptr;
    bool w_integral = false;
    unsigned char* w8 = nullptr;
    unsigned char* w8_main = nullptr;
    double* like_w = nullptr;
    double* w_main = nullptr;
    bool w_main_integral = false;
    double w_sum = 0, w_main_sum = 0;
    int w_sel = 0;
    bool borrowed = false;
    long long* wcum = nullptr;
    std::shared_ptr<BucketCols> bq;
    int64_t N = 0, n = 0, ld = 0;
    void* scratch = nullptr;
    int64_t scratch_bytes = 0;
    void* scratch2 = nullptr;
    int64_t scratch2_bytes = 0;
    void* gather_index = nullptr;
    int64_t gather_index_bytes = 0;
    FftPlanCache* fft = nullptr;
    std::map<int, double*> dctmat;
    std::map<int, void*> fft_tw;
    struct StageSlot {
        void* host = nullptr;
        size_t cap = 0;
        hipEvent_t ev = nullptr;
        bool used = false;
        bool own = false;
    };
    static constexpr size_t kStageBytes = 64u << 10;
    void* stage_block = nullptr;
    static constexpr int kCopyMarks = 16;
    hipEvent_t copy_marks[kCopyMarks] = {};
    int copy_mark_next = 0;
    static constexpr int kStageSlots = 32;
    StageSlot stage[kStageSlots];
    int stage_next = 0;
    struct Fetch {
        void* dst;
        size_t off, bytes;
    };
    static constexpr size_t kFetchBytes = 4u << 20, kFetchMax = 1u << 20;
    void* fetch_block = nullptr;
    size_t fetch_off = 0;
    std::vector<Fetch> fetch_pending;
    static constexpr int kKoptEvents = 32;
    hipEvent_t kopt_evs[kKoptEvents] = {};
    int kopt_ev_next = 0;
    void* comm = nullptr;
    int comm_world = 0, comm_rank = 0;
    void* comm_buf = nullptr;
    size_t comm_buf_bytes = 0;
    std::atomic<int> comm_abandon_gen{0};
    int comm_completed = 0;
    void* batch_state = nullptr;
    void (*batch_state_release)(gd_ctx*, bool destroy) = nullptr;
};

int gd_stage_h2d(gd_ctx* ctx, void* d_dst, const void* src, size_t bytes);
int gd_h2d(gd_ctx* ctx, void* d_dst, const void* src, size_t bytes);

int gd_fft_r2c_2d(gd_ctx* ctx, int n0, int n1, int batch, const double* d_in, double2* d_out);
int gd_fft_c2r_2d(gd_ctx* ctx, int n0, int n1, int batch, double2* d_in, double* d_out);
void gd_fft_cache_destroy(gd_ctx* ctx);

int gd_fetch(gd_ctx* ctx, void* host_dst, const void* d_src, size_t bytes);
int gd_fetch_pinned(gd_ctx* ctx, void* pinned_dst, const void* d_src, size_t bytes);
int gd_stream_sync(gd_ctx* ctx);

int gd_fail(gd_ctx* ctx, int code, const char* fmt, ...);
void gd_comm_release(gd_ctx* ctx);
bool gd_ctx_alive(gd_ctx* ctx);
int gd_stream_priority(gd_ctx* ctx, int level);
void* gd_scratch(gd_ctx* ctx, int64_t bytes);
void* gd_scratch2(gd_ctx* ctx, int64_t bytes);

#define GD_HIP(call)                                                                                 \
    do {                                                                                             \
        hipError_t e__ = (call);                                                                     \
        if (e__ != hipSuccess)                                                                       \
            return gd_fail(ctx, e__ == hipErrorOutOfMemory ? GD_ERR_NOMEM : GD_ERR_HIP, "%s: %s (%s:%d)", #call, \
                           hipGetErrorString(e__), __FILE__, __LINE__);                              \
    } while (0)

#define GD_KERNEL_CHECK() GD_HIP(hipGetLastError())

#define GD_TRY(call)              \
    do {                          \
        const int rc__ = (call);  \
        if (rc__) return rc__;    \
    } while (0)

#define GD_REQUIRE(cond, msg)                                   \
    do {                                                        \
        if (!(cond)) return gd_fail(ctx, GD_ERR_BADARG, "%s", msg); \
    } while (0)

#define WAVE 64

typedef double gd_f64x2 __attribute__((ext_vector_type(2)));
typedef unsigned int gd_u32x4 __attribute__((ext_vector_type(4)));
__device__ __forceinline__ double2 gload_d2(const double* p) {
    const gd_f64x2 v = *(const __attribute__((address_space(1))) gd_f64x2*)p;
    return make_double2(v.x, v.y);
}
__device__ __forceinline__ uint4 gload_u4(const void* p) {
    const gd_u32x4 v = *(const __attribute__((address_space(1))) gd_u32x4*)p;
    return make_uint4(v.x, v.y, v.z, v.w);
}

__device__ __forceinline__ double wave_sum(double v) {
#pragma unroll
    for (int o = 32; o > 0; o >>= 1) v += __shfl_down(v, o, WAVE);
    return v;
}
__device__ __forceinline__ double wave_min(double v) {
#pragma unroll
    for (int o = 32; o > 0; o >>= 1) v = fmin(v, __shfl_down(v, o, WAVE));
    return v;
}
__device__ __forceinline__ double wave_max(double v) {
#pragma unroll
    for (int o = 32; o > 0; o >>= 1) v = fmax(v, __shfl_down(v, o, WAVE));
    return v;
}

__device__ __forceinline__ double block_sum(double v, double* red) {
    v = wave_sum(v);
    const int lane = threadIdx.x & 63, wv = threadIdx.x >> 6, nw = (blockDim.x + 63) >> 6;
    __syncthreads();
    if (lane == 0) red[wv] = v;
    __syncthreads();
    double r = 0;
    if (threadIdx.x == 0)
        for (int i = 0; i < nw; ++i) r += red[i];
    return r;
}
__device__ __forceinline__ double block_min(double v, double* red) {
    v = wave_min(v);
    const int lane = threadIdx.x & 63, wv = threadIdx.x >> 6, nw = (blockDim.x + 63) >> 6;
    __syncthreads();
    if (lane == 0) red[wv] = v;
    __syncthreads();
    double r = red[0];
    if (threadIdx.x == 0)
        for (int i = 1; i < nw; ++i) r = fmin(r, red[i]);
    return r;
}
__device__ __forceinline__ double block_max(double v, double* red) {
    v = wave_max(v);
    const int lane = threadIdx.x & 63, wv = threadIdx.x >> 6, nw = (blockDim.x + 63) >> 6;
    __syncthreads();
    if (lane == 0) red[wv] = v;
    __syncthreads();
    double r = red[0];
    if (threadIdx.x == 0)
        for (int i = 1; i < nw; ++i) r = fmax(r, red[i]);
    return r;
}
```

### getdist_amd/csrc/kopt2d.hip

```cpp
#include "ctx.hpp"
#include "ldsfft.hpp"
#include "solvers.hpp"

#ifndef KT
#define KT 512
#endif
#define MAXF 6
#ifdef KOPT_PROFILE
__device__ long long g_prof[8];
__device__ long long g_wave[8];
#define PROF_T0 long long prof_t0 = clock64()
#define PROF_ADD(slot)                                                        \
    do {                                                                      \
        const long long prof_t1 = clock64();                                  \
        if (threadIdx.x == 0 && blockIdx.x == 0) g_prof[slot] += prof_t1 - prof_t0; \
        prof_t0 = prof_t1;                                                    \
    } while (0)
#else
#define PROF_T0
#define PROF_ADD(slot)
#endif
#ifndef KOPT_U
#define KOPT_U 1
#endif
#define KOPT_STRIDE 12
#define PI 3.141592653589793238462643383279502884
#define PISQ (PI * PI)

typedef double gd_f64x4 __attribute__((ext_vector_type(4)));
template <int EPI>
__global__ void __launch_bounds__(256) k_gemm_nt(const double* __restrict__ A, int64_t strideA,
                                                 const double* __restrict__ Bm, int64_t strideB, int F,
                                                 double* __restrict__ Cm, int64_t strideC,
                                                 const double* __restrict__ sums) {
    constexpr int KC = 32;
    __shared__ double As[KC][65];
    __shared__ double Bs[KC][65];
    const int b = blockIdx.z;
    const double* Ab = A + (int64_t)b * strideA;
    const double* Bb = Bm + (int64_t)b * strideB;
    const int i0 = blockIdx.y * 64, j0 = blockIdx.x * 64;
    const int lane = threadIdx.x & 63, wave = threadIdx.x >> 6;
    const int wi = (wave >> 1) * 32, wj = (wave & 1) * 32;
    const int l15 = lane & 15, lk = lane >> 4;
    gd_f64x4 acc[2][2];
#pragma unroll
    for (int u = 0; u < 2; ++u)
#pragma unroll
        for (int v = 0; v < 2; ++v) acc[u][v] = (gd_f64x4){0.0, 0.0, 0.0, 0.0};
    constexpr int NQ = 64 * KC / 256;
    double ra[NQ], rb[NQ];
    auto fetch = [&](int p0) {
#pragma unroll
        for (int q = 0; q < NQ; ++q) {
            const int e = threadIdx.x + 256 * q;
            const int pp = e & (KC - 1), ii = e / KC;
            const int p = p0 + pp;
            ra[q] = (i0 + ii < F && p < F) ? Ab[(int64_t)(i0 + ii) * F + p] : 0.0;
            rb[q] = (j0 + ii < F && p < F) ? Bb[(int64_t)(j0 + ii) * F + p] : 0.0;
        }
    };
    fetch(0);
    for (int p0 = 0; p0 < F; p0 += KC) {
        __syncthreads();
#pragma unroll
        for (int q = 0; q < NQ; ++q) {
            const int e = threadIdx.x + 256 * q;
            As[e & (KC - 1)][e / KC] = ra[q];
            Bs[e & (KC - 1)][e / KC] = rb[q];
        }
        __syncthreads();
        if (p0 + KC < F) fetch(p0 + KC);
#pragma unroll
        for (int kk = 0; kk < KC / 4; ++kk) {
            const int k = kk * 4 + lk;
            const double a0 = As[k][wi + l15], a1 = As[k][wi + 16 + l15];
            const double b0 = Bs[k][wj + l15], b1 = Bs[k][wj + 16 + l15];
            acc[0][0] = __builtin_amdgcn_mfma_f64_16x16x4f64(a0, b0, acc[0][0], 0, 0, 0);
            acc[0][1] = __builtin_amdgcn_mfma_f64_16x16x4f64(a0, b1, acc[0][1], 0, 0, 0);
            acc[1][0] = __builtin_amdgcn_mfma_f64_16x16x4f64(a1, b0, acc[1][0], 0, 0, 0);
            acc[1][1] = __builtin_amdgcn_mfma_f64_16x16x4f64(a1, b1, acc[1][1], 0, 0, 0);
        }
    }
    double* Cb = Cm + (int64_t)b * strideC;
    const double inv = (EPI == 1) ? sums[b] : 1.0;
#pragma unroll
    for (int u = 0; u < 2; ++u)
#pragma unroll
        for (int v = 0; v < 2; ++v)
#pragma unroll
            for (int r = 0; r < 4; ++r) {
                const int i = i0 + wi + u * 16 + lk + 4 * r, j = j0 + wj + v * 16 + l15;
                if (i < F && j < F) {
                    if (EPI == 0) {
                        Cb[(int64_t)i * F + j] = acc[u][v][r];
                    } else {
                        const double val = acc[u][v][r] / inv;
                        Cb[(int64_t)j * F + i] = val * val;
                    }
                }
            }
}


template <int EPI, bool BIG>
__global__ void __launch_bounds__(512) k_dct_pass(const double* __restrict__ src, int F, FftDev plH, const double2* __restrict__ twg,
                                                  const double2* __restrict__ cg, const double* __restrict__ sums,
                                                  double* __restrict__ dst) {
    extern __shared__ double2 dsh[];
    const int H = F >> 1, b = blockIdx.y, RPB = blockDim.x / FT;
    double2* tw = dsh;
    double2* ck = dsh + F;
    const int g = threadIdx.x / FT, t = threadIdx.x % FT;
    double2* buf = dsh + 2 * F + (size_t)g * F;
    double* stage = (double*)(buf + H);
    const int row = blockIdx.x * RPB + g;
    const bool active = row < F;
    {
        const double* x = src + (int64_t)b * F * F + (int64_t)min(row, F - 1) * F;
        for (int i0 = t; i0 < F; i0 += 8 * FT) {
            double xv[8];
#pragma unroll
            for (int q = 0; q < 8; ++q) xv[q] = x[min(i0 + q * FT, F - 1)];
            __builtin_amdgcn_sched_barrier(0);
#pragma unroll
            for (int q = 0; q < 8; ++q) stage[min(i0 + q * FT, F - 1)] = xv[q];
        }
        for (int i0 = threadIdx.x; i0 < F; i0 += 2 * blockDim.x) {
            const int i1 = min(i0 + (int)blockDim.x, F - 1);
            const double2 a0 = twg[i0], a1 = twg[i1], c0 = cg[i0], c1 = cg[i1];
            __builtin_amdgcn_sched_barrier(0);
            tw[i0] = a0, tw[i1] = a1, ck[i0] = c0, ck[i1] = c1;
        }
    }
    __syncthreads();
    if (active) {
        auto v = [&](int m) { return m < H ? stage[2 * m] : stage[2 * (F - 1 - m) + 1]; };
        for (int n = t; n < H; n += FT) buf[n] = make_double2(v(2 * n), v(2 * n + 1));
    }
    group_sync();
    fft_full<BIG, false>(buf, tw, 2, plH, t);
    if (active) {
        const double inv = EPI == 1 ? sums[b] : 1.0;
        auto put = [&](int k, double y) {
            if (EPI == 1) {
                const double val = y / inv;
                stage[k] = val * val;
            } else {
                stage[k] = y;
            }
        };
        for (int k = t; 2 * k <= H; k += FT) {
            if (k == 0) {
                const double2 z = buf[0];
                put(0, 2.0 * (z.x + z.y));
                const double vh = z.x - z.y;
                put(H, 2.0 * (ck[H].x * vh));
                continue;
            }
            const double2 zk = buf[k], zm = buf[H - k];
            const double ax = zk.x + zm.x, ay = zk.y - zm.y, bx = zk.x - zm.x, by = zk.y + zm.y;
            {
                const double2 e = tw[k];
                const double u = fma(e.x, bx, -(e.y * by)), w = fma(e.x, by, e.y * bx);
                const double vx = 0.5 * (ax + w), vy = 0.5 * (ay - u);
                const double2 c1 = ck[k], c2 = ck[F - k];
                put(k, 2.0 * fma(c1.x, vx, -(c1.y * vy)));
                put(F - k, 2.0 * fma(c2.x, vx, c2.y * vy));
            }
            if (2 * k < H) {
                const double2 f = tw[H - k];
                const double u2 = -fma(f.x, bx, f.y * by), w2 = fma(f.x, by, -(f.y * bx));
                const double vx = 0.5 * (ax + w2), vy = 0.5 * (-ay - u2);
                const double2 c1 = ck[H - k], c2 = ck[H + k];
                put(H - k, 2.0 * fma(c1.x, vx, -(c1.y * vy)));
                put(H + k, 2.0 * fma(c2.x, vx, c2.y * vy));
            }
        }
    }
    __syncthreads();
    double* out = dst + (int64_t)b * F * F + (int64_t)blockIdx.x * RPB;
    const int nrows = min(RPB, F - blockIdx.x * RPB);
    for (int e = threadIdx.x; e < F * RPB; e += blockDim.x) {
        const int k = e / RPB, r = e - k * RPB;
        if (r < nrows) {
            const double* st = (const double*)(dsh + 2 * F + (size_t)r * F + H);
            out[(int64_t)k * F + r] = st[k];
        }
    }
}

__global__ void k_dct_matrix(int F, double* __restrict__ D) {
    const int e = blockIdx.x * blockDim.x + threadIdx.x;
    if (e >= F * F) return;
    const int k = e / F, n = e % F;
    const long long m = ((long long)k * (2 * n + 1)) % (4LL * F);
    const int q = (int)(m / F);
    const int r = (int)(m - (long long)q * F);
    const double c = cospi((double)r / (2.0 * F)), s = sinpi((double)r / (2.0 * F));
    double v = (q == 0) ? c : (q == 1) ? -s : (q == 2) ? -c : s;
    D[e] = 2.0 * v;
}

__global__ void k_hist_sums(const double* __restrict__ hist, int FF, double* __restrict__ sums) {
    __shared__ double red[16];
    const double* h = hist + (int64_t)blockIdx.x * FF;
    double s = 0;
    for (int i = threadIdx.x; i < FF; i += blockDim.x) s += h[i];
    s = block_sum(s, red);
    if (threadIdx.x == 0) sums[blockIdx.x] = s;
}

__global__ void k_gather_norm(const double* __restrict__ hist, const int* __restrict__ which, const double* __restrict__ sums,
                              int FF, double* __restrict__ out) {
    const int b = which[blockIdx.y];
    const double s = sums[b];
    for (int i = blockIdx.x * blockDim.x + threadIdx.x; i < FF; i += gridDim.x * blockDim.x)
        out[(int64_t)blockIdx.y * FF + i] = hist[(int64_t)b * FF + i] / s;
}

__global__ void k_power_full(const double2* __restrict__ Z, int F, double* __restrict__ out) {
    const int Fh = F / 2 + 1;
    const double2* Zb = Z + (int64_t)blockIdx.y * F * Fh;
    double* ob = out + (int64_t)blockIdx.y * F * F;
    for (int e = blockIdx.x * blockDim.x + threadIdx.x; e < F * F; e += gridDim.x * blockDim.x) {
        const int i = e / F, j = e % F;
        double2 z;
        if (j < Fh)
            z = Zb[(int64_t)i * Fh + j];
        else
            z = Zb[(int64_t)((F - i) % F) * Fh + (F - j)];
        ob[e] = z.x * z.x + z.y * z.y;
    }
}

struct KoptLds {
    double* wx;
    double* wy;
    double* res;
    double* red;
    double* times;
    double* scale;
    double* tile;
    int tile_doubles;
};

__device__ void bilinear_forms_reg(const double* __restrict__ M, int F, int m, KoptLds L, int kmax);

__device__ void bilinear_forms(const double* __restrict__ M, int F, int m, KoptLds L, int kmax) {
    if (L.tile == nullptr) {
        bilinear_forms_reg(M, F, m, L, kmax);
        return;
    }
    const int lane = threadIdx.x & 63, wave = threadIdx.x >> 6;
    const int nseg = (kmax + 127) >> 7;
    const int rows_fit = L.tile_doubles / (nseg * 128);
    const int jx = threadIdx.x & 127, g = threadIdx.x >> 7;
    double val[MAXF];
#pragma unroll
    for (int q = 0; q < MAXF; ++q) val[q] = 0;
    PROF_T0;
    for (int r0 = 0; r0 < kmax; r0 += rows_fit) {
        const int nr = min(rows_fit, kmax - r0);
        for (int idx = wave; idx < nr * nseg; idx += KT / 64) {
            const int row = idx / nseg, seg = idx - row * nseg;
            __builtin_amdgcn_global_load_lds(
                (const __attribute__((address_space(1))) void*)(M + (int64_t)(r0 + row) * F + seg * 128 + lane * 2),
                (__attribute__((address_space(3))) void*)(L.tile + idx * 128), 16, 0, 0);
        }
        __syncthreads();
        PROF_ADD(1);
        for (int j0 = 0; j0 < nseg * 128; j0 += 256) {
            const int j = j0 + 2 * jx;
            if (j < kmax) {
                double ax[MAXF], ay[MAXF];
#pragma unroll
                for (int q = 0; q < MAXF; ++q) ax[q] = ay[q] = 0;
                const double* col = L.tile + (j >> 7) * 128 + (j & 127);
                for (int r = 2 * g; r < nr; r += 2 * (KT / 128)) {
                    const double2 a0 = *reinterpret_cast<const double2*>(col + r * nseg * 128);
                    const bool two = r + 1 < nr;
                    const double2 a1 = two ? *reinterpret_cast<const double2*>(col + (r + 1) * nseg * 128)
                                           : make_double2(0.0, 0.0);
#pragma unroll
                    for (int q = 0; q < MAXF; ++q)
                        if (q < m) {
                            const double2 wyq = *reinterpret_cast<const double2*>(L.wy + q * F + r0 + r);
                            ax[q] = fma(wyq.x, a0.x, ax[q]);
                            ay[q] = fma(wyq.x, a0.y, ay[q]);
                            const double wy1 = two ? wyq.y : 0.0;
                            ax[q] = fma(wy1, a1.x, ax[q]);
                            ay[q] = fma(wy1, a1.y, ay[q]);
                        }
                }
#pragma unroll
                for (int q = 0; q < MAXF; ++q)
                    if (q < m) {
                        val[q] = fma(ax[q], L.wx[q * F + j], val[q]);
                        if (j + 1 < kmax) val[q] = fma(ay[q], L.wx[q * F + j + 1], val[q]);
                    }
            }
        }
        __syncthreads();
        PROF_ADD(2);
    }
    const int wv = wave;
#pragma unroll
    for (int q = 0; q < MAXF; ++q)
        if (q < m) {
            const double r = wave_sum(val[q]);
            if (lane == 0) L.wx[q * 16 + wv] = r;
        }
    __syncthreads();
    if ((int)threadIdx.x < m) {
        double r = 0;
        for (int i = 0; i < KT / 64; ++i) r += L.wx[threadIdx.x * 16 + i];
        L.res[threadIdx.x] = r;
    }
    __syncthreads();
    PROF_ADD(3);
}

__device__ void bilinear_forms_reg(const double* __restrict__ M, int F, int m, KoptLds L, int kmax) {
    constexpr int U = KOPT_U;
    const int jx = threadIdx.x & 127, g = threadIdx.x >> 7;
    const int rows_per = (kmax + KT / 128 - 1) / (KT / 128);
    const int r_lo = g * rows_per, r_hi = min(kmax, r_lo + rows_per);
    double val[MAXF];
#pragma unroll
    for (int q = 0; q < MAXF; ++q) val[q] = 0;
    for (int j0 = 0; j0 < kmax; j0 += 256) {
        const int j = j0 + 2 * jx;
        if (j < kmax) {
            double ax[MAXF], ay[MAXF];
#pragma unroll
            for (int q = 0; q < MAXF; ++q) ax[q] = ay[q] = 0;
            for (int i = r_lo; i < r_hi; i += U) {
                double2 a[U];
#pragma unroll
                for (int u = 0; u < U; ++u)
                    a[u] = (i + u < r_hi) ? *reinterpret_cast<const double2*>(M + (int64_t)(i + u) * F + j)
                                          : make_double2(0.0, 0.0);
#pragma unroll
                for (int u = 0; u < U; ++u) {
                    const int iu = min(i + u, r_hi - 1);
#pragma unroll
                    for (int q = 0; q < MAXF; ++q)
                        if (q < m) {
                            const double wyq = L.wy[q * F + iu];
                            ax[q] = fma(wyq, a[u].x, ax[q]);
                            ay[q] = fma(wyq, a[u].y, ay[q]);
                        }
                }
            }
#pragma unroll
            for (int q = 0; q < MAXF; ++q)
                if (q < m) {
                    val[q] = fma(ax[q], L.wx[q * F + j], val[q]);
                    if (j + 1 < kmax) val[q] = fma(ay[q], L.wx[q * F + j + 1], val[q]);
                }
        }
    }
    __syncthreads();
    const int lane = threadIdx.x & 63, wv = threadIdx.x >> 6;
#pragma unroll
    for (int q = 0; q < MAXF; ++q)
        if (q < m) {
            const double r = wave_sum(val[q]);
            if (lane == 0) L.wx[q * 16 + wv] = r;
        }
    __syncthreads();
// ... 574 lines not shown
            wxs[idx] = v;
            wys[(mf - 1 - q) * KR_F + k] = v;
        } else {
            (isy ? wys : wxs)[idx] = v;
        }
    }
}

template <bool ODD>
__global__ void __launch_bounds__(KR_T) k_kopt2d_res(const double* __restrict__ M_all, const KoptPair* __restrict__ pairs,
                                                     double* __restrict__ out) {
    extern __shared__ double lds[];
    KresView V;
    V.wxs = lds;
    V.wys = lds + MAXF * KR_F;
    V.mt = V.wys + MAXF * KR_F;
    V.logI = V.mt + 8 * KR_LDS * KR_F;
    V.sh = reinterpret_cast<KresShared*>(V.logI + KR_F);
    KresShared* S = V.sh;
    const int b = blockIdx.x, w = threadIdx.x >> 6, l = threadIdx.x & 63;
    double* o = out + (int64_t)b * KOPT_STRIDE;
    if (ODD && !(pairs[b].do_corr && o[7] == (double)GD_OK)) return;
    double m[KR_REG][4];
    RPROF_T0;
    kres_load(M_all + (int64_t)(ODD ? pairs[b].pw_index : b) * KR_F * KR_F, m, V.mt, w, l);
    if (!ODD) {
        if (threadIdx.x < 6) S->scale[threadIdx.x] = pow(PI, (double)(2 * threadIdx.x));
        if (threadIdx.x >= 64 && threadIdx.x < 64 + 5 * MAXF) {
            const int Ls = (threadIdx.x - 64) / MAXF, a = (threadIdx.x - 64) % MAXF;
            if (a <= Ls) {
                const double cst = (1.0 + pow(0.5, (double)(Ls + 1))) / 3.0;
                S->ceven[Ls][a] = -2.0 * cst * k_even(a) * k_even(Ls - a);
            }
        }
        if (threadIdx.x >= 256) V.logI[threadIdx.x - 256] = log((double)(threadIdx.x - 256) * (double)(threadIdx.x - 256));
    } else {
        if (threadIdx.x >= 8 && threadIdx.x < 14) S->scale[threadIdx.x - 2] = pow(2.0 * PI, (double)(2 * (threadIdx.x - 8)));
        if (threadIdx.x >= 128 && threadIdx.x < 138) S->kodd[threadIdx.x - 128] = k_odd(threadIdx.x - 128);
        if (threadIdx.x >= 192 && threadIdx.x < 195) {
            const int Ls = 4 + 2 * (threadIdx.x - 192);
            S->codd[threadIdx.x - 192] = 8.0 * (1.0 - pow(2.0, (double)(-Ls - 1))) / 3.0;
        }
    }
    if (threadIdx.x == 0) {
        const KoptPair P = pairs[b];
        S->N = P.N, S->fallback_t = P.fallback_t, S->do_corr = P.do_corr;
        S->xpre = 0.0, S->xcur = 0.1, S->xblk = 0.0, S->fblk = 0.0, S->spre = 0.0, S->scur = 0.0, S->t_star = 0.0;
        S->fpre = 0.0, S->fcur = 0.0;
        S->status = GD_OK, S->done = 0, S->it = -2;
        S->x = 0.0;
        if (!ODD) {
            S->stage = KR_STAGE_BRENT, S->Ls = 5, S->Lmin = 2, S->t = 0.0;
        } else {
            S->stage = KR_STAGE_ODD, S->Ls = 10, S->Lmin = 4, S->t = o[0];
            S->p00 = o[4];
        }
        for (int q = 0; q < MAXF; ++q) S->times[q] = S->t;
    }
    for (int e = threadIdx.x; e < 6 * MAXF; e += KR_T) (&S->lev[0][0])[e] = 0.0;
#ifdef KOPT_PROFILE
    if (threadIdx.x < 8) S->prof[threadIdx.x] = 0, S->wave_cycles[threadIdx.x] = 0;
#endif
    __syncthreads();
    RPROF_ADD(1);
#pragma unroll 1
    for (;;) {
        const int stage = S->stage, Ls = S->Ls;
        if (stage == KR_STAGE_EXIT) break;
        const int mf = ODD ? Ls / 2 : Ls + 1;
        kres_weights<ODD>(V.wxs, V.wys, V.logI, S->times, Ls, mf, Ls == (ODD ? 10 : 5), threadIdx.x);
        RPROF_ADD(0);
        __syncthreads();
        RPROF_ADD(5);
        kres_forms(m, V, mf, w, l);
        __syncthreads();
        RPROF_ADD(3);
        if (threadIdx.x < MAXF) kres_tail<ODD>(S, Ls, threadIdx.x);
        RPROF_ADD(7);
        __syncthreads();
        RPROF_ADD(4);
    }
#ifdef KOPT_PROFILE
    if (threadIdx.x < 8 && blockIdx.x == 0 && !ODD) g_prof[threadIdx.x] += S->prof[threadIdx.x], g_wave[threadIdx.x] += S->wave_cycles[threadIdx.x];
#endif
    if (threadIdx.x == 0) {
        if (!ODD) {
            const bool ok = S->status == GD_OK;
            const bool dc = ok && S->do_corr;
            o[0] = ok ? S->t_star : NAN;
            o[1] = ok ? S->lev[2][0] : NAN, o[2] = ok ? S->lev[2][2] : NAN, o[3] = ok ? S->lev[2][1] : NAN;
            o[4] = dc ? S->lev[0][0] : NAN;
            o[5] = NAN, o[6] = NAN;
            o[7] = (double)S->status;
        } else {
            o[5] = S->odd[0][0];
            o[6] = S->odd[0][1];
        }
    }
}

__global__ void __launch_bounds__(64) k_get_h(double* __restrict__ kopt, const double* __restrict__ neff,
                                              const double* __restrict__ corr, const int* __restrict__ do_corr, int B) {
    const int b = blockIdx.x;
    if (b >= B || threadIdx.x >= 4) return;
    double* o = kopt + (int64_t)b * KOPT_STRIDE;
    const bool ok = o[7] == (double)GD_OK;
    double psi[6];
    for (int q = 0; q < 6; ++q) psi[q] = o[1 + q];
    if (!ok) {
        if (threadIdx.x == 0) o[8] = o[9] = o[10] = NAN, o[11] = (double)GD_ERR_SOLVER;
        return;
    }
    const gdsolve::GetHResult r = gdsolve::get_h(psi, neff[b], corr[b], do_corr[b] != 0);
    if (threadIdx.x == 0) {
        o[8] = r.hx, o[9] = r.hy, o[10] = r.corr;
        o[11] = r.status ? (double)GD_ERR_BADARG : (double)GD_OK;
    }
}

extern "C" {

int gd_get_h(gd_ctx* ctx, int32_t B, const double* psi, const double* neff, const double* corr, const int32_t* do_corr,
             double* out) {
    GD_REQUIRE(ctx && psi && neff && corr && do_corr && out && B > 0, "bad argument");
    int64_t off = 0;
    auto take = [&](int64_t bytes) {
        int64_t o = off;
        off += (bytes + 255) / 256 * 256;
        return o;
    };
    const int64_t o_k = take((int64_t)B * KOPT_STRIDE * 8), o_n = take((int64_t)B * 8), o_c = take((int64_t)B * 8),
                  o_d = take((int64_t)B * 4);
    char* base = (char*)gd_scratch(ctx, off);
    if (!base) return GD_ERR_NOMEM;
    std::vector<double> hk((size_t)B * KOPT_STRIDE, 0.0);
    for (int b = 0; b < B; ++b) {
        for (int q = 0; q < 6; ++q) hk[(size_t)b * KOPT_STRIDE + 1 + q] = psi[(size_t)b * 6 + q];
        hk[(size_t)b * KOPT_STRIDE + 7] = (double)GD_OK;
    }
    GD_TRY(gd_h2d(ctx, base + o_k, hk.data(), hk.size() * 8));
    GD_TRY(gd_h2d(ctx, base + o_n, neff, (size_t)B * 8));
    GD_TRY(gd_h2d(ctx, base + o_c, corr, (size_t)B * 8));
    GD_TRY(gd_h2d(ctx, base + o_d, do_corr, (size_t)B * 4));
    k_get_h<<<B, 64, 0, ctx->stream>>>((double*)(base + o_k), (const double*)(base + o_n), (const double*)(base + o_c),
                                      (const int*)(base + o_d), B);
    GD_KERNEL_CHECK();
    GD_TRY(gd_fetch(ctx, hk.data(), base + o_k, hk.size() * 8));
    GD_TRY(gd_stream_sync(ctx));
    for (int b = 0; b < B; ++b)
        for (int q = 0; q < 4; ++q) out[(size_t)b * 4 + q] = hk[(size_t)b * KOPT_STRIDE + 8 + q];
    return GD_OK;
}

static int kopt_stage_a(gd_ctx* ctx, int32_t B, int32_t F, const void* d_hist_v, const double* neff, const int32_t* do_corr,
                        const double* fallback_t, double* d_rows) {
    GD_REQUIRE(ctx && d_hist_v && neff && do_corr && fallback_t && d_rows && B > 0, "bad argument");
    GD_REQUIRE(F >= 16 && F <= 1024, "KernelOptimizer2D grid size out of range (16..1024)");
    const double* d_hist = (const double*)d_hist_v;
    const int64_t FF = (int64_t)F * F;
    FftDev plH;
    const double2 *d_tw = nullptr, *d_ck = nullptr;
    bool dct_fft = F % 2 == 0 && F / 2 <= 512 && F >= 64 && getenv("GDHIP_KOPT_DCT_GEMM") == nullptr &&
                   lds_fft_plan(ctx, F / 2, &plH, nullptr);
    if (dct_fft) {
        FftDev plF;
        dct_fft = lds_fft_plan(ctx, F, &plF, &d_tw);
    }
    if (dct_fft) {
        auto it = ctx->fft_tw.find(-F);
        if (it == ctx->fft_tw.end()) {
            std::vector<double2> hck((size_t)F);
            for (int k = 0; k < F; ++k) {
                const long double a = -3.141592653589793238462643383279502884L * (long double)k / (2.0L * (long double)F);
                hck[k] = make_double2((double)cosl(a), (double)sinl(a));
            }
            void* d = nullptr;
            GD_HIP(hipMalloc(&d, (size_t)F * 16));
            if (hipMemcpy(d, hck.data(), (size_t)F * 16, hipMemcpyHostToDevice) != hipSuccess) {
                (void)hipFree(d);
                return gd_fail(ctx, GD_ERR_HIP, "upload of the DCT post-twiddles failed");
            }
            it = ctx->fft_tw.emplace(-F, d).first;
        }
        d_ck = (const double2*)it->second;
    }
    double* D = nullptr;
    if (!dct_fft) {
        auto it = ctx->dctmat.find(F);
        if (it == ctx->dctmat.end()) {
            GD_HIP(hipMalloc((void**)&D, (size_t)FF * 8));
            k_dct_matrix<<<(unsigned)((FF + 255) / 256), 256, 0, ctx->stream>>>(F, D);
            GD_KERNEL_CHECK();
            ctx->dctmat[F] = D;
        } else {
            D = it->second;
        }
    }
    std::vector<KoptPair> hp((size_t)B);
    std::vector<int> which;
    for (int b = 0; b < B; ++b) {
        hp[b].N = neff[b];
        hp[b].fallback_t = fallback_t[b];
        hp[b].do_corr = do_corr[b] ? 1 : 0;
        hp[b].pw_index = -1;
        if (do_corr[b]) {
            hp[b].pw_index = (int)which.size();
            which.push_back(b);
        }
    }
    const int nc = (int)which.size();
    const int Fh = F / 2 + 1;
    int64_t off = 0;
    auto take = [&](int64_t bytes) {
        int64_t o = off;
        off += (bytes + 255) / 256 * 256;
        return o;
    };
    const int64_t o_pairs = take((int64_t)B * sizeof(KoptPair)), o_which = take((int64_t)(nc + 1) * 4);
    const int64_t table_bytes = off;
    const int64_t o_sums = take((int64_t)B * 8), o_E = take((int64_t)B * FF * 8),
                  o_SQ = take((int64_t)B * FF * 8), o_Z = take((int64_t)nc * F * Fh * 16), o_PW = take((int64_t)nc * FF * 8);
    char* base = (char*)gd_scratch(ctx, off);
    if (!base) return GD_ERR_NOMEM;
    double* d_sums = (double*)(base + o_sums);
    KoptPair* d_pairs = (KoptPair*)(base + o_pairs);
    double* d_out = d_rows;
    int* d_which = (int*)(base + o_which);
    double* d_E = (double*)(base + o_E);
    double* d_SQ = (double*)(base + o_SQ);
    double2* d_Z = (double2*)(base + o_Z);
    double* d_PW = (double*)(base + o_PW);
    {
        std::vector<char> tab((size_t)table_bytes, 0);
        memcpy(tab.data() + o_pairs, hp.data(), (size_t)B * sizeof(KoptPair));
        if (nc) memcpy(tab.data() + o_which, which.data(), (size_t)nc * 4);
        GD_TRY(gd_stage_h2d(ctx, base, tab.data(), (size_t)table_bytes));
    }
    k_hist_sums<<<B, 1024, 0, ctx->stream>>>(d_hist, (int)FF, d_sums);
    GD_KERNEL_CHECK();
    if (dct_fft) {
        const int RPB = F <= 256 ? 16 : (F <= 512 ? 8 : 4);
        const size_t lds = ((size_t)2 * F + (size_t)RPB * F) * 16;
        const dim3 grid((F + RPB - 1) / RPB, B);
        const bool big = F / 2 > 320;
        auto k0 = big ? k_dct_pass<0, true> : k_dct_pass<0, false>;
        auto k1 = big ? k_dct_pass<1, true> : k_dct_pass<1, false>;
        GD_HIP(hipFuncSetAttribute((const void*)k0, hipFuncAttributeMaxDynamicSharedMemorySize, (int)lds));
        GD_HIP(hipFuncSetAttribute((const void*)k1, hipFuncAttributeMaxDynamicSharedMemorySize, (int)lds));
        k0<<<grid, RPB * FT, lds, ctx->stream>>>(d_hist, F, plH, d_tw, d_ck, nullptr, d_E);
        GD_KERNEL_CHECK();
        k1<<<grid, RPB * FT, lds, ctx->stream>>>(d_E, F, plH, d_tw, d_ck, d_sums, d_SQ);
        GD_KERNEL_CHECK();
    } else {
        const dim3 ggrid((F + 63) / 64, (F + 63) / 64, B);
        k_gemm_nt<0><<<ggrid, 256, 0, ctx->stream>>>(D, 0, d_hist, FF, F, d_E, FF, nullptr);
        GD_KERNEL_CHECK();
        k_gemm_nt<1><<<ggrid, 256, 0, ctx->stream>>>(d_E, FF, D, 0, F, d_SQ, FF, d_sums);
        GD_KERNEL_CHECK();
    }
    if (nc > 0) {
        k_gather_norm<<<dim3(64, nc), 256, 0, ctx->stream>>>(d_hist, d_which, d_sums, (int)FF, d_E);
        GD_KERNEL_CHECK();
        int rc = gd_fft_r2c_2d(ctx, F, F, nc, d_E, d_Z);
        if (rc) return rc;
        k_power_full<<<dim3(64, nc), 256, 0, ctx->stream>>>(d_Z, F, d_PW);
        GD_KERNEL_CHECK();
    }
    const size_t lds_base = ((size_t)2 * MAXF * F + 8 + 16 + 8 + 16) * 8;
    size_t tile_bytes = 0;
    if (F % 128 == 0 && getenv("GDHIP_KOPT_NO_LDS_TILE") == nullptr) {
        const size_t room = (size_t)160 * 1024 - 1024 - lds_base;
        size_t cap = (size_t)128 * 1024;
        if (const char* e = getenv("GDHIP_KOPT_TILE_KB")) cap = (size_t)atoi(e) * 1024;
        tile_bytes = room < cap ? room : cap;
        tile_bytes = tile_bytes / ((size_t)F * 8) * ((size_t)F * 8);
    }
    const size_t lds = lds_base + tile_bytes;
    if (F == KR_F && getenv("GDHIP_KOPT_STREAMED") == nullptr) {
        const size_t lds_res = ((size_t)2 * MAXF * KR_F + (size_t)8 * KR_LDS * KR_F + KR_F) * 8 + sizeof(KresShared);
        GD_HIP(hipFuncSetAttribute((const void*)k_kopt2d_res<false>, hipFuncAttributeMaxDynamicSharedMemorySize, (int)lds_res));
        k_kopt2d_res<false><<<B, KR_T, lds_res, ctx->stream>>>(d_SQ, d_pairs, d_out);
        if (nc > 0) {
            GD_KERNEL_CHECK();
            GD_HIP(hipFuncSetAttribute((const void*)k_kopt2d_res<true>, hipFuncAttributeMaxDynamicSharedMemorySize, (int)lds_res));
            k_kopt2d_res<true><<<B, KR_T, lds_res, ctx->stream>>>(d_PW, d_pairs, d_out);
        }
    } else {
        GD_HIP(hipFuncSetAttribute((const void*)k_kopt2d, hipFuncAttributeMaxDynamicSharedMemorySize, (int)lds));
        k_kopt2d<<<B, KT, lds, ctx->stream>>>(d_SQ, d_PW, d_pairs, F, (int)(tile_bytes / 8), d_out);
    }
    GD_KERNEL_CHECK();
#ifdef KOPT_PROFILE
    {
        long long hp[8];
        GD_TRY(gd_stream_sync(ctx));
        GD_HIP(hipMemcpyFromSymbol(hp, HIP_SYMBOL(g_prof), sizeof(hp)));
        fprintf(stderr, "kopt block 0 cycles: weights %lld  tile-load %lld  tile-fma %lld  reduce %lld  "
                        "entry-barrier %lld  times/pow %lld | levels (streamed) or barrier after the weights (resident) %lld  kmax sum %lld\n",
                hp[0], hp[1], hp[2], hp[3], hp[4], hp[7], hp[5], hp[6]);
        long long hw[8];
        GD_HIP(hipMemcpyFromSymbol(hw, HIP_SYMBOL(g_wave), sizeof(hw)));
        fprintf(stderr, "  forms per wave: %lld %lld %lld %lld %lld %lld %lld %lld\n", hw[0], hw[1], hw[2], hw[3], hw[4], hw[5], hw[6], hw[7]);
        memset(hp, 0, sizeof(hp));
        GD_HIP(hipMemcpyToSymbol(HIP_SYMBOL(g_prof), hp, sizeof(hp)));
        GD_HIP(hipMemcpyToSymbol(HIP_SYMBOL(g_wave), hp, sizeof(hp)));
    }
#endif
    return GD_OK;
}

#define KOPT_BLOCK_DOUBLES 15
static int kopt_stage_b(gd_ctx* ctx, hipEvent_t after, int32_t B, double* d_rows, double* out) {
    GD_REQUIRE(ctx && d_rows && out && B > 0, "bad argument");
    if (after) GD_HIP(hipStreamWaitEvent(ctx->stream, after, 0));
    const double* d_neff = d_rows + (int64_t)B * KOPT_STRIDE;
    const double* d_corr = d_neff + B;
    const int* d_dc = (const int*)(d_corr + B);
    k_get_h<<<B, 64, 0, ctx->stream>>>(d_rows, d_neff, d_corr, d_dc, B);
    GD_KERNEL_CHECK();
    GD_TRY(gd_fetch(ctx, out, d_rows, (size_t)B * KOPT_STRIDE * 8));
    GD_TRY(gd_stream_sync(ctx));
    return GD_OK;
}

static int kopt_upload_get_h_inputs(gd_ctx* ctx, int32_t B, double* d_rows, const double* neff, const double* corr,
                                    const int32_t* do_corr) {
    std::vector<double> tab((size_t)3 * B, 0.0);
    memcpy(tab.data(), neff, (size_t)B * 8);
    memcpy(tab.data() + B, corr, (size_t)B * 8);
    memcpy(tab.data() + 2 * (size_t)B, do_corr, (size_t)B * 4);
    return gd_h2d(ctx, d_rows + (int64_t)B * KOPT_STRIDE, tab.data(), tab.size() * 8);
}

int gd_kopt2d(gd_ctx* ctx, int32_t B, int32_t F, const void* d_hist_v, const double* neff, const int32_t* do_corr,
              const double* fallback_t, const double* corr, double* out) {
    GD_REQUIRE(ctx && d_hist_v && neff && do_corr && fallback_t && corr && out && B > 0, "bad argument");
    double* d_rows = (double*)gd_scratch2(ctx, (int64_t)B * KOPT_BLOCK_DOUBLES * 8);
    if (!d_rows) return GD_ERR_NOMEM;
    GD_TRY(kopt_upload_get_h_inputs(ctx, B, d_rows, neff, corr, do_corr));
    GD_TRY(kopt_stage_a(ctx, B, F, d_hist_v, neff, do_corr, fallback_t, d_rows));
    return kopt_stage_b(ctx, nullptr, B, d_rows, out);
}

int gd_kopt2d_enqueue(gd_ctx* ctx, int32_t B, int32_t F, const void* d_hist, const double* neff, const int32_t* do_corr,
                      const double* fallback_t, const double* corr, void* d_rows, int32_t* ticket_out) {
    GD_REQUIRE(ctx && ticket_out && d_rows && neff && corr && do_corr && B > 0, "bad argument");
    GD_TRY(kopt_upload_get_h_inputs(ctx, B, (double*)d_rows, neff, corr, do_corr));
    GD_TRY(kopt_stage_a(ctx, B, F, d_hist, neff, do_corr, fallback_t, (double*)d_rows));
    const int slot = ctx->kopt_ev_next;
    ctx->kopt_ev_next = (slot + 1) % gd_ctx::kKoptEvents;
    if (!ctx->kopt_evs[slot]) GD_HIP(hipEventCreateWithFlags(&ctx->kopt_evs[slot], hipEventDisableTiming));
    GD_HIP(hipEventRecord(ctx->kopt_evs[slot], ctx->stream));
    *ticket_out = slot;
    return GD_OK;
}

int gd_kopt2d_finish(gd_ctx* ctx, gd_ctx* stage_a_ctx, int32_t ticket, int32_t B, void* d_rows, double* out) {
    GD_REQUIRE(ctx && stage_a_ctx && ticket >= 0 && ticket < gd_ctx::kKoptEvents && stage_a_ctx->kopt_evs[ticket], "bad ticket");
    GD_HIP(hipSetDevice(ctx->device));
    return kopt_stage_b(ctx, ctx == stage_a_ctx ? nullptr : stage_a_ctx->kopt_evs[ticket], B, (double*)d_rows, out);
}

}
```

### include/gdhip.h

```cpp
#ifndef GDHIP_H
#define GDHIP_H

#include <stdint.h>

#ifdef __cplusplus
extern "C" {
#endif

typedef struct gd_ctx gd_ctx;

typedef enum gd_status {
    GD_OK = 0,
    GD_ERR_BADARG = -1,
    GD_ERR_NOMEM = -2,
    GD_ERR_HIP = -3,
    GD_ERR_EMPTY = -4,
    GD_ERR_SOLVER = -5,
    GD_ERR_FFT = -6,
    GD_ERR_NODEVICE = -7,
    GD_ERR_TIMEOUT = -8
} gd_status;

int gd_device_count(void);
int gd_create(int device, gd_ctx** out);
void gd_destroy(gd_ctx* ctx);
const char* gd_last_error(gd_ctx* ctx);
const char* gd_version(void);
int gd_device_info(gd_ctx* ctx, int64_t* info6);
int gd_sync(gd_ctx* ctx);
int gd_dev_alloc(gd_ctx* ctx, int64_t bytes, void** d_out);
int gd_dev_free(gd_ctx* ctx, void* d_ptr);
int gd_memcpy_h2d(gd_ctx* ctx, void* d_dst, const void* src, int64_t bytes);
int gd_memcpy_d2h(gd_ctx* ctx, void* dst, const void* d_src, int64_t bytes);
int gd_memcpy_d2h_async(gd_ctx* ctx, void* dst, const void* d_src, int64_t bytes);
int gd_copy_sync(gd_ctx* ctx);
int gd_copy_mark(gd_ctx* ctx, int32_t* token_out);
int gd_copy_wait(gd_ctx* ctx, int32_t token);
int gd_memcpy_d2d(gd_ctx* ctx, void* d_dst, const void* d_src, int64_t bytes);
int gd_memset(gd_ctx* ctx, void* d_dst, int value, int64_t bytes);
int gd_gather_items(gd_ctx* ctx, void* d_dst, const void* d_src, const int32_t* index, int32_t count, int64_t item_bytes);
int gd_host_alloc(gd_ctx* ctx, int64_t bytes, void** out);
int gd_host_free(gd_ctx* ctx, void* ptr);
int gd_timer_start(gd_ctx* ctx);
int gd_timer_stop_ms(gd_ctx* ctx, double* ms_out);

int gd_upload(gd_ctx* ctx, const double* X, int64_t N, int64_t n, int64_t row_stride, int64_t col_stride,
              const double* weights);
int gd_num_rows(gd_ctx* ctx, int64_t* N, int64_t* n);
int gd_column_ptr(gd_ctx* ctx, int64_t j, void** d_out);

int gd_weight_stats(gd_ctx* ctx, int64_t row_lo, int64_t row_hi, double thresh, double* out4);
int gd_col_stats(gd_ctx* ctx, int64_t row_lo, int64_t row_hi, double* out);
int gd_cov(gd_ctx* ctx, const int32_t* cols, int32_t m, int64_t row_lo, int64_t row_hi, double* means_out,
           double* cov_out, double* norm_out, double* minmax_out);

int gd_quantiles(gd_ctx* ctx, const int32_t* cols, int32_t ncols, int64_t row_lo, int64_t row_hi,
                 const double* targets, int32_t k, double* out);

int gd_quantiles_mm(gd_ctx* ctx, const int32_t* cols, int32_t ncols, int64_t row_lo, int64_t row_hi,
                    const double* targets, int32_t k, const double* minmax, double* out);

int gd_quantiles_mm_probe(gd_ctx* ctx, const int32_t* cols, int32_t ncols, int64_t row_lo, int64_t row_hi,
                          const double* targets, int32_t k, const double* minmax, double* out, const double* probe_means,
                          double* probe_out, int32_t* probe_done);

int gd_autocov_lags(gd_ctx* ctx, int32_t col, double mean, int64_t k0, int32_t nlags, double* out);
int gd_kde_lag_sums(gd_ctx* ctx, int32_t col, double inv4s2, const int64_t* lags, int32_t nlags, double* out);
int gd_kde_lag_sums_2d(gd_ctx* ctx, int32_t coli, int32_t colj, const double* kinv3, const int64_t* lags, int32_t nlags,
                       double* out);
int gd_autocov_lags_batch(gd_ctx* ctx, const int32_t* cols, int32_t ncols, const double* means, int64_t k0,
                          int32_t nlags, double* out);
int gd_kde_lag_sums_batch(gd_ctx* ctx, const int32_t* cols, int32_t ncols, const double* inv4s2, const int64_t* lags,
                          int32_t nlags, double* out);
int gd_autocov_lags_range_batch(gd_ctx* ctx, const int32_t* cols, int32_t ncols, const double* means, int64_t row_lo,
                                int64_t row_hi, int64_t k0, int32_t nlags, double* out);

int gd_hist1d(gd_ctx* ctx, const int32_t* cols, int32_t ncols, const double* binmin, const double* width,
              int32_t F, double* out);
int gd_hist1d_dev(gd_ctx* ctx, const int32_t* cols, int32_t ncols, const double* binmin, const double* width,
                  int32_t F, void* d_out);
int gd_bin_indices(gd_ctx* ctx, int32_t col, double binmin, double width, int32_t round_half, int32_t F,
                   int32_t* idx_out, int64_t* n_out_of_range);
int gd_prebin(gd_ctx* ctx, int32_t col, double binmin, double width, int32_t F, void* d_idx_u16);
int gd_prebin8_batch(gd_ctx* ctx, const int32_t* cols, int32_t ncols, const double* binmin, const double* width, int32_t F,
                     void* const* d_idx_out, int64_t* bad_out);
int gd_hist2d_prebinned8(gd_ctx* ctx, int32_t B, const void* const* d_idx_x, const void* const* d_idx_y, void* d_hist);
int gd_prebin8_hist2d(gd_ctx* ctx, const int32_t* cols, int32_t ncols, const double* binmin, const double* width,
                      void* const* d_idx_out, int64_t* bad_out, int32_t B, const void* const* d_idx_x,
                      const void* const* d_idx_y, void* d_hist);

int gd_prebin_batch(gd_ctx* ctx, const int32_t* cols, int32_t ncols, const double* binmin, const double* width, int32_t F,
                    void* const* d_idx_u16);
int gd_hist2d(gd_ctx* ctx, int32_t B, const int32_t* colx, const int32_t* coly, const double* binminx,
              const double* widthx, const double* binminy, const double* widthy, int32_t F, void* d_hist);
int gd_hist2d_prebinned(gd_ctx* ctx, int32_t B, const void* const* d_idx_x, const void* const* d_idx_y, int32_t F,
                        void* d_hist);
int gd_minmax_affine(gd_ctx* ctx, int32_t B, const int32_t* coli, const int32_t* colj, const double* a,
                     const double* b, double* out);
int gd_hist2d_sheared(gd_ctx* ctx, int32_t B, const int32_t* coli, const int32_t* colj, const double* r0,
                      const double* r1, const double* xmin, const double* dx, const double* ymin, const double* dy,
                      int32_t F, void* d_hist);

int gd_isj1d(gd_ctx* ctx, int32_t B, int32_t F, const double* hist, const double* neff, double* hfrac_out,
             int32_t* status_out);
int gd_isj1d_dev(gd_ctx* ctx, int32_t B, int32_t F, const void* d_hist, const double* neff, double* hfrac_out,
                 int32_t* status_out);

int gd_dct1d(gd_ctx* ctx, int32_t B, int32_t F, const double* hist, double* a_out);
int gd_density1d(gd_ctx* ctx, int32_t B, int32_t F, const double* hist, const double* smooth, const int32_t* winw,
                 const int32_t* flags, int32_t bco, int32_t mbc, double* P_out, int32_t* status_out);
int gd_density1d_dev(gd_ctx* ctx, int32_t B, int32_t F, const void* d_hist, const double* smooth, const int32_t* winw,
                     const int32_t* flags, int32_t bco, int32_t mbc, double* P_out, int32_t* status_out);

int gd_kopt2d(gd_ctx* ctx, int32_t B, int32_t F, const void* d_hist, const double* neff, const int32_t* do_corr,
              const double* fallback_t, const double* corr, double* out);
#define GD_KOPT_BLOCK_DOUBLES 15
int gd_kopt2d_enqueue(gd_ctx* ctx, int32_t B, int32_t F, const void* d_hist, const double* neff, const int32_t* do_corr,
                      const double* fallback_t, const double* corr, void* d_rows, int32_t* ticket_out);
int gd_kopt2d_finish(gd_ctx* ctx, gd_ctx* stage_a_ctx, int32_t ticket, int32_t B, void* d_rows, double* out);
int gd_get_h(gd_ctx* ctx, int32_t B, const double* psi, const double* neff, const double* corr, const int32_t* do_corr,
             double* out);

int gd_density2d(gd_ctx* ctx, int32_t B, int32_t F, const void* d_hist, const double* rx, const double* ry,
                 const double* corr, const int32_t* winw, const int32_t* flags, int32_t bco, int32_t mbc,
                 void* d_P_out, int32_t* status_out);
int gd_density2d_enqueue(gd_ctx* ctx, int32_t B, int32_t F, const void* d_hist, const double* rx, const double* ry,
                         const double* corr, const int32_t* winw, const int32_t* flags, int32_t bco, int32_t mbc,
                         void* d_P_out, int32_t* status_pinned);

int gd_density2d_enqueue_indexed(gd_ctx* ctx, int32_t B, int32_t F, const void* d_hist, const int32_t* hist_index,
                                 const double* rx, const double* ry, const double* corr, const int32_t* winw,
                                 const int32_t* flags, int32_t bco, int32_t mbc, void* d_P_out, int32_t* status_pinned);

int gd_attach_samples(gd_ctx* ctx, gd_ctx* owner);
int gd_bind_thread(gd_ctx* ctx);

int gd_contour_levels(gd_ctx* ctx, int32_t B, int32_t F, const void* d_P, const double* contours, int32_t nc, double* out,
                      int32_t* status_out);

int gd_limits1d(gd_ctx* ctx, int32_t B, int32_t F, const double* P, const double* x0, const double* spacing,
                const double* contours, int32_t nc, int32_t factor, double* out, int32_t* status_out);

int gd_set_extra_column(gd_ctx* ctx, int32_t slot, const double* x);
int gd_aux_weights(gd_ctx* ctx, const double* w);
int gd_col_minmax(gd_ctx* ctx, const int32_t* cols, int32_t ncols, int64_t lo, int64_t hi, int32_t cond_col,
                  double cond_below, double* out);

int gd_weights_integral(gd_ctx* ctx, int32_t* out);
int gd_thin_rows(gd_ctx* ctx, int64_t lo, int64_t hi, int64_t factor, int32_t unique_mode, void* d_rows, int64_t capacity,
                 int64_t* count_out);
int gd_binary_transitions(gd_ctx* ctx, const int32_t* cols, int32_t ncols, const void* d_rows, int64_t K,
                          const double* thresholds, int32_t nthr, int64_t* counts_out);
int gd_thinned_lag_sums(gd_ctx* ctx, const int32_t* cols, int32_t ncols, const double* means, const void* d_rows, int64_t K,
                        int32_t maxoff, double* out);

int gd_like_weights(gd_ctx* ctx, const double* loglikes, int32_t mode, double mean_loglike, double* sum_out);
int gd_select_weights(gd_ctx* ctx, int32_t which);
int gd_likes1d(gd_ctx* ctx, int32_t B, int32_t F, const double* hist, const double* likehist, const double* P,
               const double* smooth, const int32_t* winw, const int32_t* flags, int32_t shade_mean_loglikes,
               double* likes_out, int32_t* status_out);
int gd_likes2d(gd_ctx* ctx, int32_t B, int32_t F, const void* d_hist, const void* d_likehist, const double* rx,
               const double* ry, const double* corr, const int32_t* winw, const int32_t* flags, int32_t mbc,
               void* d_likes_out, int32_t* status_out);

int gd_density2d_masked(gd_ctx* ctx, int32_t F, const void* d_hist, double rx, double ry, double corr, int32_t winw,
                        int32_t flags, int32_t bco, int32_t mbc, const double* mask_bc, const double* mask_mbc,
                        const unsigned char* zero_mask, void* d_P_out, int32_t* status_out);

#define GD_HISTND_MAXD 25
#define GD_HISTND_MAX_BINS (1 << 25)
#define GD_HISTND_H 1
#define GD_HISTND_LIKES 2
#define GD_HISTND_LMIN 4
int gd_histnd_batch(gd_ctx* ctx, int32_t B, const int32_t* dims, const int32_t* cols, const double* binmin,
                    const double* width, int32_t nb, int32_t flags, int32_t loglike_col, double* H_out, double* HL_out,
                    double* Lmin_out);

#define GD_PCA_MAX_PROJ 448
int gd_pca_corr(gd_ctx* ctx, const int32_t* cols, int32_t n, const int32_t* maps, double* mean_out, double* sd_out,
                double* corr_out);
int gd_pca_project(gd_ctx* ctx, const int32_t* cols, int32_t np, const int32_t* maps, const double* mean, const double* sd,
                   const double* U, int32_t doexp, int32_t n_all, const double* all_means, const double* all_sd,
                   double* newmean_out, double* newsd_out, double* pcpc_out, double* pcpar_out);

int gd_mixture_nll(gd_ctx* ctx, const int32_t* cols, int32_t d, int32_t K, const double* means, const double* whiten,
                   const double* logcoef, int64_t row_lo, int64_t row_hi, double* out);

int gd_circ_convolve(gd_ctx* ctx, int32_t n0, int32_t n1, const double* a, const double* b, double* out);
int gd_convolve1d_direct(gd_ctx* ctx, const double* x, int64_t nx, const double* y, int64_t ny, double* out_full);
int gd_autoconvolve(gd_ctx* ctx, int32_t col, double mean, int32_t use_weights, const double* x_host, int64_t nx, int64_t s,
                    int64_t n, int32_t normalize, double* out);

int gd_like_stats(gd_ctx* ctx, int32_t col, double* out8);


#define GD_BATCH2D_META 32
#define GD_BATCH2D_NEED_NEFF (-20)

typedef struct gd_param2d {
    double range_min, range_max;
    double param_min, param_max;
    double sigma_range, err;
    double mean, var;
    double neff;
    int32_t has_limits_bot, has_limits_top, periodic;
    int32_t owned;
} gd_param2d;

typedef struct gd_batch2d_settings {
    int32_t fine_bins_2D, boundary_correction_order, mult_bias_correction_order, num_bins_2D;
    double smooth_scale_2D, max_corr_2D;
    double norm, sum_w2;
    int32_t uncorrelated_sampler;
    int32_t raise_on_bandwidth_errors;
    int32_t want_levels, ncontours;
    const double* contours;
    int32_t two_streams_min;
    int32_t two_streams_split;
    int32_t kopt_split_min;
    double kopt_first_fraction;
    int32_t first_batch, max_batch;
    double max_batch_bytes;
    int32_t comm_exchange;
    int32_t bandwidths_only;
    const double* pair_neff;
    const double* bandwidths;
    int32_t results_in_flight;
} gd_batch2d_settings;

typedef int (*gd_neff_exchange_fn)(void* user, double* neff_n, int32_t n);

int gd_batch2d_grid_sizes(const gd_batch2d_settings* settings, int32_t n, const double* corr, const int32_t* pairs,
                          int32_t P, int32_t* F_out);
int gd_density2d_batch(gd_ctx* ctx, gd_ctx* twin, const gd_batch2d_settings* settings, gd_param2d* params, int32_t n,
                       const double* corr, const double* cov, const double* lag_probe, const int32_t* pairs, int32_t P,
                       gd_neff_exchange_fn exchange, void* exchange_user, void* grids_pinned, int64_t grids_doubles,
                       int32_t* status_pinned, double* meta, double* levels, int32_t* level_status, int32_t* tokens_out2);
#define GD_BATCH1D_META 9

typedef struct gd_density1d_settings {
    int32_t fine_bins, num_bins, boundary_correction_order, mult_bias_correction_order;
    double smooth_scale_1D;
    double norm, sum_w2;
    int32_t uncorrelated_sampler;
    int32_t raise_on_bandwidth_errors;
} gd_density1d_settings;

int gd_density1d_batch(gd_ctx* ctx, const gd_density1d_settings* settings, gd_param2d* params, int32_t n, const int32_t* cols,
                       int32_t B, double* P_out, double* hist_out, double* meta);

int gd_batch2d_finish(gd_ctx* ctx);
int gd_batch2d_invalidate(gd_ctx* ctx);
int gd_batch2d_exchanges(gd_ctx* ctx, int64_t* count_out);


int gd_comm_rccl_path(char* buf, int32_t len, int32_t* preloaded_out);
int gd_upload_shard(gd_ctx* ctx, const double* X_cols, int64_t N, int64_t n, int64_t col_first, int64_t col_count,
                    int64_t col_stride, const double* weights);
int gd_comm_share_columns(gd_ctx* ctx, const int64_t* first_by_rank );
int gd_comm_unique_id(void* id128_out);
int gd_comm_init(gd_ctx* ctx, int32_t world, int32_t rank, const void* id128);
int gd_comm_info(gd_ctx* ctx, int32_t* world_out, int32_t* rank_out);
int gd_comm_abandon(gd_ctx* ctx);
int gd_comm_destroy(gd_ctx* ctx);
int gd_comm_allgather(gd_ctx* ctx, const double* send, int64_t count, double* recv);
int gd_comm_allreduce_sum(gd_ctx* ctx, double* inout, int64_t count);
int gd_comm_allgather_dev(gd_ctx* ctx, const void* d_send, int64_t count, void* d_recv);
int gd_comm_allreduce_sum_dev(gd_ctx* ctx, const void* d_send, int64_t count, void* d_recv);

#ifdef __cplusplus
}
#endif
// ... 2 lines not shown
```

Measured before the change: 50860.

## Read kopt histograms through a pointer table and fuse normalisation sums into the first pass

The 2D kernel-optimiser stage no longer gathers the rotated and pairwise histograms into one contiguous pool buffer. It passes a per-batch table of row pointers that the DCT, GEMM, sums and gather kernels dereference directly. For count-weighted histograms, the per-histogram sums are accumulated with atomics inside the first DCT/GEMM pass, which removes the separate k_hist_sums launch. The spectrum branch is also deferred until after the first resident kopt kernel. The aim is to cut a device-to-device copy and a full read pass per batch, at the cost of atomics, pointer indirection and an extra finish call in the copy_sync path, which looks questionable.

```diff
diff --git a/getdist_amd/_lib.py b/getdist_amd/_lib.py
--- a/getdist_amd/_lib.py
+++ b/getdist_amd/_lib.py
@@ -96,6 +96,9 @@
     "gd_kopt2d": (C.c_int, [_p, _i32, _i32, _p, _pd, _pi32, _pd, _pd, _pd]),
     "gd_kopt2d_enqueue": (C.c_int, [_p, _i32, _i32, _p, _pd, _pi32, _pd, _pd, _p, _pi32]),
     "gd_kopt2d_finish": (C.c_int, [_p, _p, _i32, _i32, _p, _pd]),
+    "gd_kopt2d_rows": (C.c_int, [_p, _i32, _i32, _p, _p, _i32, _pd, _pi32, _pd, _pd, _pd]),
+    "gd_kopt2d_enqueue_rows": (C.c_int, [_p, _i32, _i32, _p, _p, _i32, _pd, _pi32, _pd, _pd, _p, _pi32]),
+    "gd_kopt2d_last_sums": (C.c_int, [_p, _i32, _pd]),
     "gd_get_h": (C.c_int, [_p, _i32, _pd, _pd, _pd, _pi32, _pd]),
     "gd_density2d": (C.c_int, [_p, _i32, _i32, _p, _pd, _pd, _pd, _pi32, _pi32, _i32, _i32, _p, _pi32]),
     "gd_copy_mark": (C.c_int, [_p, _pi32]),
@@ -877,6 +880,23 @@
         self._check(self.lib.gd_batch2d_exchanges(self.h, C.byref(c)))
         return int(c.value)
 
+    def kopt2d_rows(self, rows, B, F, neff, do_corr, fallback_t, corr, counts=False):
+        neff, do_corr, fallback_t, corr = _f64arr(neff), _i32arr(do_corr), _f64arr(fallback_t), _f64arr(corr)
+        out = np.zeros((B, 12))
+        if isinstance(rows, DevBuf):
+            d_hist, table = rows.ptr, None
+        else:
+            assert len(rows) == B
+            d_hist, table = None, (_p * B)(*[int(r) for r in rows])
+        self._check(self.lib.gd_kopt2d_rows(self.h, B, F, d_hist, table, 1 if counts else 0, _dp(neff), _ip(do_corr),
+                                            _dp(fallback_t), _dp(corr), _dp(out)))
+        return out
+
+    def kopt2d_last_sums(self, B):
+        out = np.zeros(B)
+        self._check(self.lib.gd_kopt2d_last_sums(self.h, B, _dp(out)))
+        return out
+
     def kopt2d(self, d_hist, B, F, neff, do_corr, fallback_t, corr):
         neff, do_corr, fallback_t, corr = _f64arr(neff), _i32arr(do_corr), _f64arr(fallback_t), _f64arr(corr)
         out = np.zeros((B, 12))
diff --git a/getdist_amd/csrc/batch2d.hip b/getdist_amd/csrc/batch2d.hip
--- a/getdist_amd/csrc/batch2d.hip
+++ b/getdist_amd/csrc/batch2d.hip
@@ -96,6 +96,19 @@
      [](void* ctx, int level) { return gd_stream_priority(C(ctx), level); },
     [](void* h, const int32_t* cols, int32_t ncols, const double* binmin, const double* width, int32_t F, void* const* d_idx) {
         return gd_prebin_batch(C(h), cols, ncols, binmin, width, F, d_idx);
+    },
+};
+
+const gdb::OpsRows kOpsRows = {
+    [](void* h, int32_t B, int32_t F, const void* d_hist, const void* const* rows, int32_t counts, const double* neff,
+       const int32_t* do_corr, const double* fallback_t, const double* corr, double* out) {
+        const int32_t flags = (counts || C(h)->w == nullptr || C(h)->w8 != nullptr) ? GD_KOPT_COUNTS : 0;
+        return gd_kopt2d_rows(C(h), B, F, d_hist, rows, flags, neff, do_corr, fallback_t, corr, out);
+    },
+    [](void* h, int32_t B, int32_t F, const void* d_hist, const void* const* rows, int32_t counts, const double* neff,
+       const int32_t* do_corr, const double* fallback_t, const double* corr, void* d_rows, int32_t* ticket) {
+        const int32_t flags = (counts || C(h)->w == nullptr || C(h)->w8 != nullptr) ? GD_KOPT_COUNTS : 0;
+        return gd_kopt2d_enqueue_rows(C(h), B, F, d_hist, rows, flags, neff, do_corr, fallback_t, corr, d_rows, ticket);
     },
 };
 
@@ -164,6 +177,8 @@
     try {
         gdb::Call call(state_of(ctx), kOps, ctx, twin, *settings, params, n, corr, cov, lag_probe, pairs, P, exchange, exchange_user,
                        (double*)grids_pinned, grids_doubles, status_pinned, meta, levels, level_status);
+        const char* sw = getenv("GDHIP_KOPT_GATHER");
+        call.rows_ops = (sw != nullptr && atoi(sw) != 0) ? nullptr : &kOpsRows;
         rc = call.run(tokens_out2);
         if (rc) ctx->err = call.err;
     } catch (const std::exception& e) {
diff --git a/getdist_amd/csrc/batch2d.hpp b/getdist_amd/csrc/batch2d.hpp
--- a/getdist_amd/csrc/batch2d.hpp
+++ b/getdist_amd/csrc/batch2d.hpp
@@ -70,6 +70,14 @@
                         void* const* d_idx);
 };
 
+struct OpsRows {
+    int (*kopt2d_rows)(void* h, int32_t B, int32_t F, const void* d_hist, const void* const* rows, int32_t counts,
+                       const double* neff, const int32_t* do_corr, const double* fallback_t, const double* corr, double* out);
+    int (*kopt2d_enqueue_rows)(void* h, int32_t B, int32_t F, const void* d_hist, const void* const* rows, int32_t counts,
+                               const double* neff, const int32_t* do_corr, const double* fallback_t, const double* corr,
+                               void* d_rows, int32_t* ticket);
+};
+
 static inline double py_pow(double x, double y) {
     volatile double e = y;
     return pow(x, e);
@@ -427,6 +435,7 @@
           pairs(pairs_), P(P_), exchange(ex_), exchange_user(ex_user_), grids(grids_), grids_doubles(grids_doubles_),
           status_pinned(status_), meta(meta_), levels(levels_), level_status(level_status_), pool{st_, ops_, h_} {}
 
+    const OpsRows* rows_ops = nullptr;
     int64_t N = 0;
     bool unit_weights = true;
     Pool pool;
@@ -1087,6 +1096,7 @@
         bool whole = false;
         void* d_batch = nullptr;
         bool own = false;
+        std::vector<const void*> src;
         void* d_rows = nullptr;
         int32_t ticket = -1;
         std::vector<double> ne, fb, ci;
@@ -1116,7 +1126,13 @@
         const int B = (int)L.ks.size(), F = L.F;
         const int64_t item = (int64_t)F * F * 8;
         L.d_batch = L.d_hist, L.own = false;
-        if (!L.whole) {
+        L.src.clear();
+        if (!L.whole && rows_ops) {
+            L.d_batch = nullptr;
+            L.src.reserve(B);
+            for (int a = 0; a < L.na; ++a) L.src.push_back((const char*)shear.d_rot + (int64_t)a * item);
+            for (int q : L.pos) L.src.push_back((const char*)L.d_hist + (int64_t)q * item);
+        } else if (!L.whole) {
             int rc = 0;
             L.d_batch = pool.take((int64_t)B * item, &rc);
             if (!L.d_batch) return dev_fail(rc, h);
@@ -1297,7 +1313,11 @@
                 std::vector<double> out((size_t)B * 12);
                 if (!rc) {
                     mark("kopt: launch", B, L.F);
-                    rc = ops.kopt2d(h, B, L.F, L.d_batch, L.ne.data(), L.dc.data(), L.fb.data(), L.ci.data(), out.data());
+                    if (rows_ops)
+                        rc = rows_ops->kopt2d_rows(h, B, L.F, L.d_batch, L.src.empty() ? nullptr : L.src.data(), unit_weights ? 1 : 0,
+                                                   L.ne.data(), L.dc.data(), L.fb.data(), L.ci.data(), out.data());
+                    else
+                        rc = ops.kopt2d(h, B, L.F, L.d_batch, L.ne.data(), L.dc.data(), L.fb.data(), L.ci.data(), out.data());
                     mark("kopt: done");
                     if (rc) dev_fail(rc, h);
                 }
@@ -1363,6 +1383,7 @@
                         if (e) dev_fail(e, aux);
                     } else {
                         ops.copy_sync(h);
+                        if (rows_ops) (void)ops.kopt2d_finish(aux, h, L.ticket, B, L.d_rows, out.data());
                     }
                     if (L.own) pool.give(L.d_batch);
                     pool.give(L.d_rows);
@@ -1386,7 +1407,12 @@
                 }
                 if (!rc) {
                     mark("kopt: stage A enqueue", q, B);
-                    rc = ops.kopt2d_enqueue(h, B, L.F, L.d_batch, L.ne.data(), L.dc.data(), L.fb.data(), L.ci.data(), L.d_rows, &L.ticket);
+                    if (rows_ops)
+                        rc = rows_ops->kopt2d_enqueue_rows(h, B, L.F, L.d_batch, L.src.empty() ? nullptr : L.src.data(),
+                                                           unit_weights ? 1 : 0, L.ne.data(), L.dc.data(), L.fb.data(),
+                                                           L.ci.data(), L.d_rows, &L.ticket);
+                    else
+                        rc = ops.kopt2d_enqueue(h, B, L.F, L.d_batch, L.ne.data(), L.dc.data(), L.fb.data(), L.ci.data(), L.d_rows, &L.ticket);
                     if (rc) dev_fail(rc, h);
                 }
                 std::lock_guard<std::mutex> g(mu);
diff --git a/getdist_amd/csrc/ctx.hpp b/getdist_amd/csrc/ctx.hpp
--- a/getdist_amd/csrc/ctx.hpp
+++ b/getdist_amd/csrc/ctx.hpp
@@ -88,6 +88,8 @@
     static constexpr int kKoptEvents = 32;
     hipEvent_t kopt_evs[kKoptEvents] = {};
     int kopt_ev_next = 0;
+    double* kopt_sums = nullptr;
+    int kopt_sums_count = 0;
     void* comm = nullptr;
     int comm_world = 0, comm_rank = 0;
     void* comm_buf = nullptr;
diff --git a/getdist_amd/csrc/kopt2d.hip b/getdist_amd/csrc/kopt2d.hip
--- a/getdist_amd/csrc/kopt2d.hip
+++ b/getdist_amd/csrc/kopt2d.hip
@@ -28,18 +28,22 @@
 #define PISQ (PI * PI)
 
 typedef double gd_f64x4 __attribute__((ext_vector_type(4)));
+typedef const __attribute__((address_space(1))) double* gd_gptr;
 template <int EPI>
 __global__ void __launch_bounds__(256) k_gemm_nt(const double* __restrict__ A, int64_t strideA,
                                                  const double* __restrict__ Bm, int64_t strideB, int F,
                                                  double* __restrict__ Cm, int64_t strideC,
-                                                 const double* __restrict__ sums) {
+                                                 const double* __restrict__ sums, const double* const* __restrict__ rowsB,
+                                                 double* __restrict__ tot) {
     constexpr int KC = 32;
     __shared__ double As[KC][65];
     __shared__ double Bs[KC][65];
     const int b = blockIdx.z;
     const double* Ab = A + (int64_t)b * strideA;
-    const double* Bb = Bm + (int64_t)b * strideB;
+    const gd_gptr Bb = (gd_gptr)(rowsB ? rowsB[b] : Bm + (int64_t)b * strideB);
     const int i0 = blockIdx.y * 64, j0 = blockIdx.x * 64;
+    const bool summing = EPI == 0 && tot != nullptr && blockIdx.y == 0;
+    double bsum = 0;
     const int lane = threadIdx.x & 63, wave = threadIdx.x >> 6;
     const int wi = (wave >> 1) * 32, wj = (wave & 1) * 32;
     const int l15 = lane & 15, lk = lane >> 4;
@@ -58,6 +62,7 @@
             const int p = p0 + pp;
             ra[q] = (i0 + ii < F && p < F) ? Ab[(int64_t)(i0 + ii) * F + p] : 0.0;
             rb[q] = (j0 + ii < F && p < F) ? Bb[(int64_t)(j0 + ii) * F + p] : 0.0;
+            if (summing) bsum += rb[q];
         }
     };
     fetch(0);
@@ -81,6 +86,10 @@
             acc[1][0] = __builtin_amdgcn_mfma_f64_16x16x4f64(a1, b0, acc[1][0], 0, 0, 0);
             acc[1][1] = __builtin_amdgcn_mfma_f64_16x16x4f64(a1, b1, acc[1][1], 0, 0, 0);
         }
+    }
+    if (summing) {
+        bsum = wave_sum(bsum);
+        if (lane == 0) atomicAdd(&tot[b], bsum);
     }
     double* Cb = Cm + (int64_t)b * strideC;
     const double inv = (EPI == 1) ? sums[b] : 1.0;
@@ -106,8 +115,11 @@
 template <int EPI, bool BIG>
 __global__ void __launch_bounds__(512) k_dct_pass(const double* __restrict__ src, int F, FftDev plH, const double2* __restrict__ twg,
                                                   const double2* __restrict__ cg, const double* __restrict__ sums,
-                                                  double* __restrict__ dst) {
+                                                  double* __restrict__ dst, const double* const* __restrict__ rows,
+                                                  double* __restrict__ acc) {
     extern __shared__ double2 dsh[];
+    __shared__ double wsum[8];
+    const bool summing = EPI == 0 && acc != nullptr;
     const int H = F >> 1, b = blockIdx.y, RPB = blockDim.x / FT;
     double2* tw = dsh;
     double2* ck = dsh + F;
@@ -117,7 +129,8 @@
     const int row = blockIdx.x * RPB + g;
     const bool active = row < F;
     {
-        const double* x = src + (int64_t)b * F * F + (int64_t)min(row, F - 1) * F;
+        const gd_gptr x = (gd_gptr)(rows ? rows[b] : src + (int64_t)b * F * F) + (int64_t)min(row, F - 1) * F;
+        double rsum = 0;
         for (int i0 = t; i0 < F; i0 += 8 * FT) {
             double xv[8];
 #pragma unroll
@@ -125,6 +138,15 @@
             __builtin_amdgcn_sched_barrier(0);
 #pragma unroll
             for (int q = 0; q < 8; ++q) stage[min(i0 + q * FT, F - 1)] = xv[q];
+            if (summing) {
+#pragma unroll
+                for (int q = 0; q < 8; ++q)
+                    if (active && i0 + q * FT < F) rsum += xv[q];
+            }
+        }
+        if (summing) {
+            rsum = wave_sum(rsum);
+            if ((threadIdx.x & 63) == 0) wsum[threadIdx.x >> 6] = rsum;
         }
         for (int i0 = threadIdx.x; i0 < F; i0 += 2 * blockDim.x) {
             const int i1 = min(i0 + (int)blockDim.x, F - 1);
@@ -134,6 +156,11 @@
         }
     }
     __syncthreads();
+    if (summing && threadIdx.x == 0) {
+        double r = 0;
+        for (int w = 0; w < (int)(blockDim.x + 63) / 64; ++w) r += wsum[w];
+        atomicAdd(&acc[b], r);
+    }
     if (active) {
         auto v = [&](int m) { return m < H ? stage[2 * m] : stage[2 * (F - 1 - m) + 1]; };
         for (int n = t; n < H; n += FT) buf[n] = make_double2(v(2 * n), v(2 * n + 1));
@@ -202,9 +229,10 @@
     D[e] = 2.0 * v;
 }
 
-__global__ void k_hist_sums(const double* __restrict__ hist, int FF, double* __restrict__ sums) {
+__global__ void k_hist_sums(const double* __restrict__ hist, int FF, double* __restrict__ sums,
+                            const double* const* __restrict__ rows) {
     __shared__ double red[16];
-    const double* h = hist + (int64_t)blockIdx.x * FF;
+    const gd_gptr h = (gd_gptr)(rows ? rows[blockIdx.x] : hist + (int64_t)blockIdx.x * FF);
     double s = 0;
     for (int i = threadIdx.x; i < FF; i += blockDim.x) s += h[i];
     s = block_sum(s, red);
@@ -212,11 +240,18 @@
 }
 
 __global__ void k_gather_norm(const double* __restrict__ hist, const int* __restrict__ which, const double* __restrict__ sums,
-                              int FF, double* __restrict__ out) {
+                              int FF, double* __restrict__ out, const double* const* __restrict__ rows) {
     const int b = which[blockIdx.y];
     const double s = sums[b];
+    const gd_gptr h = (gd_gptr)(rows ? rows[b] : hist + (int64_t)b * FF);
     for (int i = blockIdx.x * blockDim.x + threadIdx.x; i < FF; i += gridDim.x * blockDim.x)
-        out[(int64_t)blockIdx.y * FF + i] = hist[(int64_t)b * FF + i] / s;
+        out[(int64_t)blockIdx.y * FF + i] = h[i] / s;
+}
+
+__global__ void k_gather_rows(const double* const* __restrict__ rows, int64_t item16, double2* __restrict__ dst) {
+    const double* h = rows[blockIdx.y];
+    double2* d = dst + (int64_t)blockIdx.y * item16;
+    for (int64_t i = blockIdx.x * blockDim.x + threadIdx.x; i < item16; i += (int64_t)gridDim.x * blockDim.x) d[i] = gload_d2(h + 2 * i);
 }
 
 __global__ void k_power_full(const double2* __restrict__ Z, int F, double* __restrict__ out) {
@@ -1097,10 +1132,16 @@
     return GD_OK;
 }
 
-static int kopt_stage_a(gd_ctx* ctx, int32_t B, int32_t F, const void* d_hist_v, const double* neff, const int32_t* do_corr,
-                        const double* fallback_t, double* d_rows) {
-    GD_REQUIRE(ctx && d_hist_v && neff && do_corr && fallback_t && d_rows && B > 0, "bad argument");
+static int kopt_stage_a(gd_ctx* ctx, int32_t B, int32_t F, const void* d_hist_v, const void* const* rows, int32_t flags,
+                        const double* neff, const int32_t* do_corr, const double* fallback_t, double* d_rows) {
+    GD_REQUIRE(ctx && (d_hist_v != nullptr) != (rows != nullptr) && neff && do_corr && fallback_t && d_rows && B > 0, "bad argument");
     GD_REQUIRE(F >= 16 && F <= 1024, "KernelOptimizer2D grid size out of range (16..1024)");
+    if (rows)
+        for (int b = 0; b < B; ++b) GD_REQUIRE(rows[b] && ((uintptr_t)rows[b] & 15) == 0, "a histogram pointer is null or not 16-byte aligned");
+    const char* sw = getenv("GDHIP_KOPT_GATHER");
+    const bool legacy = sw != nullptr && atoi(sw) != 0;
+    GD_REQUIRE(!(rows && legacy) || F % 2 == 0, "the gathered form needs an even grid size");
+    const bool fused_sums = (flags & GD_KOPT_COUNTS) != 0 && !legacy;
     const double* d_hist = (const double*)d_hist_v;
     const int64_t FF = (int64_t)F * F;
     FftDev plH;
@@ -1161,13 +1202,16 @@
         off += (bytes + 255) / 256 * 256;
         return o;
     };
-    const int64_t o_pairs = take((int64_t)B * sizeof(KoptPair)), o_which = take((int64_t)(nc + 1) * 4);
+    const int64_t o_pairs = take((int64_t)B * sizeof(KoptPair)), o_which = take((int64_t)(nc + 1) * 4),
+                  o_src = take(rows ? (int64_t)B * 8 : 0), o_sums = take((int64_t)B * 8);
     const int64_t table_bytes = off;
-    const int64_t o_sums = take((int64_t)B * 8), o_E = take((int64_t)B * FF * 8),
-                  o_SQ = take((int64_t)B * FF * 8), o_Z = take((int64_t)nc * F * Fh * 16), o_PW = take((int64_t)nc * FF * 8);
+    const int64_t o_E = take((int64_t)B * FF * 8), o_SQ = take((int64_t)B * FF * 8), o_Z = take((int64_t)nc * F * Fh * 16),
+                  o_PW = take((int64_t)nc * FF * 8), o_G = take(rows && legacy ? (int64_t)B * FF * 8 : 0);
     char* base = (char*)gd_scratch(ctx, off);
     if (!base) return GD_ERR_NOMEM;
     double* d_sums = (double*)(base + o_sums);
+    ctx->kopt_sums = d_sums, ctx->kopt_sums_count = B;
+    const double* const* d_src = rows ? (const double* const*)(base + o_src) : nullptr;
     KoptPair* d_pairs = (KoptPair*)(base + o_pairs);
     double* d_out = d_rows;
     int* d_which = (int*)(base + o_which);
@@ -1179,10 +1223,21 @@
         std::vector<char> tab((size_t)table_bytes, 0);
         memcpy(tab.data() + o_pairs, hp.data(), (size_t)B * sizeof(KoptPair));
         if (nc) memcpy(tab.data() + o_which, which.data(), (size_t)nc * 4);
+        if (rows) memcpy(tab.data() + o_src, rows, (size_t)B * 8);
         GD_TRY(gd_stage_h2d(ctx, base, tab.data(), (size_t)table_bytes));
     }
-    k_hist_sums<<<B, 1024, 0, ctx->stream>>>(d_hist, (int)FF, d_sums);
-    GD_KERNEL_CHECK();
+    if (rows && legacy) {
+        int bx = (int)((FF / 2 + 255) / 256);
+        if (bx > 64) bx = 64;
+        k_gather_rows<<<dim3(bx, B), 256, 0, ctx->stream>>>(d_src, FF / 2, (double2*)(base + o_G));
+        GD_KERNEL_CHECK();
+        d_hist = (const double*)(base + o_G), d_src = nullptr;
+    }
+    double* d_acc = fused_sums ? d_sums : nullptr;
+    if (!fused_sums) {
+        k_hist_sums<<<B, 1024, 0, ctx->stream>>>(d_hist, (int)FF, d_sums, d_src);
+        GD_KERNEL_CHECK();
+    }
     if (dct_fft) {
         const int RPB = F <= 256 ? 16 : (F <= 512 ? 8 : 4);
         const size_t lds = ((size_t)2 * F + (size_t)RPB * F) * 16;
@@ -1192,25 +1247,29 @@
         auto k1 = big ? k_dct_pass<1, true> : k_dct_pass<1, false>;
         GD_HIP(hipFuncSetAttribute((const void*)k0, hipFuncAttributeMaxDynamicSharedMemorySize, (int)lds));
         GD_HIP(hipFuncSetAttribute((const void*)k1, hipFuncAttributeMaxDynamicSharedMemorySize, (int)lds));
-        k0<<<grid, RPB * FT, lds, ctx->stream>>>(d_hist, F, plH, d_tw, d_ck, nullptr, d_E);
+        k0<<<grid, RPB * FT, lds, ctx->stream>>>(d_hist, F, plH, d_tw, d_ck, nullptr, d_E, d_src, d_acc);
         GD_KERNEL_CHECK();
-        k1<<<grid, RPB * FT, lds, ctx->stream>>>(d_E, F, plH, d_tw, d_ck, d_sums, d_SQ);
+        k1<<<grid, RPB * FT, lds, ctx->stream>>>(d_E, F, plH, d_tw, d_ck, d_sums, d_SQ, nullptr, nullptr);
         GD_KERNEL_CHECK();
     } else {
         const dim3 ggrid((F + 63) / 64, (F + 63) / 64, B);
-        k_gemm_nt<0><<<ggrid, 256, 0, ctx->stream>>>(D, 0, d_hist, FF, F, d_E, FF, nullptr);
+        k_gemm_nt<0><<<ggrid, 256, 0, ctx->stream>>>(D, 0, d_hist, FF, F, d_E, FF, nullptr, d_src, d_acc);
         GD_KERNEL_CHECK();
-        k_gemm_nt<1><<<ggrid, 256, 0, ctx->stream>>>(d_E, FF, D, 0, F, d_SQ, FF, d_sums);
+        k_gemm_nt<1><<<ggrid, 256, 0, ctx->stream>>>(d_E, FF, D, 0, F, d_SQ, FF, d_sums, nullptr, nullptr);
         GD_KERNEL_CHECK();
     }
-    if (nc > 0) {
-        k_gather_norm<<<dim3(64, nc), 256, 0, ctx->stream>>>(d_hist, d_which, d_sums, (int)FF, d_E);
+    auto spectrum_branch = [&]() -> int {
+        if (nc == 0) return GD_OK;
+        k_gather_norm<<<dim3(64, nc), 256, 0, ctx->stream>>>(d_hist, d_which, d_sums, (int)FF, d_E, d_src);
         GD_KERNEL_CHECK();
         int rc = gd_fft_r2c_2d(ctx, F, F, nc, d_E, d_Z);
         if (rc) return rc;
         k_power_full<<<dim3(64, nc), 256, 0, ctx->stream>>>(d_Z, F, d_PW);
         GD_KERNEL_CHECK();
-    }
+        return GD_OK;
+    };
+    const bool resident = F == KR_F && getenv("GDHIP_KOPT_STREAMED") == nullptr;
+    if (legacy || !resident) GD_TRY(spectrum_branch());
     const size_t lds_base = ((size_t)2 * MAXF * F + 8 + 16 + 8 + 16) * 8;
     size_t tile_bytes = 0;
     if (F % 128 == 0 && getenv("GDHIP_KOPT_NO_LDS_TILE") == nullptr) {
@@ -1221,12 +1280,13 @@
         tile_bytes = tile_bytes / ((size_t)F * 8) * ((size_t)F * 8);
     }
     const size_t lds = lds_base + tile_bytes;
-    if (F == KR_F && getenv("GDHIP_KOPT_STREAMED") == nullptr) {
+    if (resident) {
         const size_t lds_res = ((size_t)2 * MAXF * KR_F + (size_t)8 * KR_LDS * KR_F + KR_F) * 8 + sizeof(KresShared);
         GD_HIP(hipFuncSetAttribute((const void*)k_kopt2d_res<false>, hipFuncAttributeMaxDynamicSharedMemorySize, (int)lds_res));
         k_kopt2d_res<false><<<B, KR_T, lds_res, ctx->stream>>>(d_SQ, d_pairs, d_out);
         if (nc > 0) {
             GD_KERNEL_CHECK();
+            if (!legacy) GD_TRY(spectrum_branch());
             GD_HIP(hipFuncSetAttribute((const void*)k_kopt2d_res<true>, hipFuncAttributeMaxDynamicSharedMemorySize, (int)lds_res));
             k_kopt2d_res<true><<<B, KR_T, lds_res, ctx->stream>>>(d_PW, d_pairs, d_out);
         }
@@ -1283,15 +1343,41 @@
     double* d_rows = (double*)gd_scratch2(ctx, (int64_t)B * KOPT_BLOCK_DOUBLES * 8);
     if (!d_rows) return GD_ERR_NOMEM;
     GD_TRY(kopt_upload_get_h_inputs(ctx, B, d_rows, neff, corr, do_corr));
-    GD_TRY(kopt_stage_a(ctx, B, F, d_hist_v, neff, do_corr, fallback_t, d_rows));
+    GD_TRY(kopt_stage_a(ctx, B, F, d_hist_v, nullptr, 0, neff, do_corr, fallback_t, d_rows));
     return kopt_stage_b(ctx, nullptr, B, d_rows, out);
+}
+
+int gd_kopt2d_rows(gd_ctx* ctx, int32_t B, int32_t F, const void* d_hist, const void* const* rows, int32_t flags,
+                   const double* neff, const int32_t* do_corr, const double* fallback_t, const double* corr, double* out) {
+    GD_REQUIRE(ctx && (d_hist || rows) && neff && do_corr && fallback_t && corr && out && B > 0, "bad argument");
+    double* d_rows = (double*)gd_scratch2(ctx, (int64_t)B * KOPT_BLOCK_DOUBLES * 8);
+    if (!d_rows) return GD_ERR_NOMEM;
+    GD_TRY(kopt_upload_get_h_inputs(ctx, B, d_rows, neff, corr, do_corr));
+    GD_TRY(kopt_stage_a(ctx, B, F, d_hist, rows, flags, neff, do_corr, fallback_t, d_rows));
+    return kopt_stage_b(ctx, nullptr, B, d_rows, out);
+}
+
+int gd_kopt2d_last_sums(gd_ctx* ctx, int32_t B, double* out) {
+    GD_REQUIRE(ctx && out && B > 0, "bad argument");
+    const char* lo = (const char*)ctx->scratch;
+    GD_REQUIRE(ctx->kopt_sums && B <= ctx->kopt_sums_count && (const char*)ctx->kopt_sums >= lo &&
+                   (const char*)(ctx->kopt_sums + B) <= lo + ctx->scratch_bytes,
+               "no optimiser call whose sums are still there");
+    GD_TRY(gd_fetch(ctx, out, ctx->kopt_sums, (size_t)B * 8));
+    return gd_stream_sync(ctx);
 }
 
 int gd_kopt2d_enqueue(gd_ctx* ctx, int32_t B, int32_t F, const void* d_hist, const double* neff, const int32_t* do_corr,
                       const double* fallback_t, const double* corr, void* d_rows, int32_t* ticket_out) {
+    return gd_kopt2d_enqueue_rows(ctx, B, F, d_hist, nullptr, 0, neff, do_corr, fallback_t, corr, d_rows, ticket_out);
+}
+
+int gd_kopt2d_enqueue_rows(gd_ctx* ctx, int32_t B, int32_t F, const void* d_hist, const void* const* rows, int32_t flags,
+                           const double* neff, const int32_t* do_corr, const double* fallback_t, const double* corr,
+                           void* d_rows, int32_t* ticket_out) {
     GD_REQUIRE(ctx && ticket_out && d_rows && neff && corr && do_corr && B > 0, "bad argument");
     GD_TRY(kopt_upload_get_h_inputs(ctx, B, (double*)d_rows, neff, corr, do_corr));
-    GD_TRY(kopt_stage_a(ctx, B, F, d_hist, neff, do_corr, fallback_t, (double*)d_rows));
+    GD_TRY(kopt_stage_a(ctx, B, F, d_hist, rows, flags, neff, do_corr, fallback_t, (double*)d_rows));
     const int slot = ctx->kopt_ev_next;
     ctx->kopt_ev_next = (slot + 1) % gd_ctx::kKoptEvents;
     if (!ctx->kopt_evs[slot]) GD_HIP(hipEventCreateWithFlags(&ctx->kopt_evs[slot], hipEventDisableTiming));
diff --git a/include/gdhip.h b/include/gdhip.h
--- a/include/gdhip.h
+++ b/include/gdhip.h
@@ -118,6 +118,13 @@
 int gd_kopt2d_enqueue(gd_ctx* ctx, int32_t B, int32_t F, const void* d_hist, const double* neff, const int32_t* do_corr,
                       const double* fallback_t, const double* corr, void* d_rows, int32_t* ticket_out);
 int gd_kopt2d_finish(gd_ctx* ctx, gd_ctx* stage_a_ctx, int32_t ticket, int32_t B, void* d_rows, double* out);
+#define GD_KOPT_COUNTS 1
+int gd_kopt2d_rows(gd_ctx* ctx, int32_t B, int32_t F, const void* d_hist, const void* const* rows, int32_t flags,
+                   const double* neff, const int32_t* do_corr, const double* fallback_t, const double* corr, double* out);
+int gd_kopt2d_enqueue_rows(gd_ctx* ctx, int32_t B, int32_t F, const void* d_hist, const void* const* rows, int32_t flags,
+                           const double* neff, const int32_t* do_corr, const double* fallback_t, const double* corr,
+                           void* d_rows, int32_t* ticket_out);
+int gd_kopt2d_last_sums(gd_ctx* ctx, int32_t B, double* out);
 int gd_get_h(gd_ctx* ctx, int32_t B, const double* psi, const double* neff, const double* corr, const int32_t* do_corr,
              double* out);
 
```

Result: slower. 50300 (-1.1%).
